# cserteGT3/RANSAC.jl

Measured on AMD Instinct MI355X. Metric: candidates_scored_per_sec, higher is better.
Workload: dtype f64; 1 GPU; cfg3: 10M-point 40-primitive cloud, 30% outliers, r=32 subsets, B=4096 candidates/GPU/step; points=10000000, subset_points=312500, score_mode=f64, parallelism=candidate-sharded x1, int32 sum all-reduce

## Files before the change

### include/ransac_hip.h

```cpp
#ifndef RANSAC_HIP_H
#define RANSAC_HIP_H

#include <stdint.h>

#ifdef __cplusplus
extern "C" {
#endif

#define RH_VERSION 121

enum {
    RH_OK = 0,
    RH_E_INVALID = -1,
    RH_E_NODEVICE = -2,
    RH_E_NOMEM = -3,
    RH_E_CAPACITY = -4,
    RH_E_INTERNAL = -5,
};

enum { RH_PLANE = 0, RH_SPHERE = 1, RH_CYLINDER = 2, RH_CONE = 3 };

typedef struct {
    int32_t kind;
    int32_t outwards;
    double v[10];
} rh_shape;

enum { RH_SCORE_INT64_WRAP = 0, RH_SCORE_F64 = 1 };
enum { RH_S_LENGTHC = 1, RH_S_ALLCAND = 2, RH_S_NOFMINSET = 3 };

typedef struct {
    double eps[4];
    double alpha[4];
    double cos_alpha[4];
    double collin_threshold;
    double parallelthrdeg;
    double cos_parallelthr;
    double sphere_par;
    double minconeopang;
    double prob_det;
    int64_t tau;
    int64_t itermax;
    int32_t drawN;
    int32_t minsubsetN;
    int32_t extract_s;
    int32_t terminate_s;
    int32_t n_shape_types;
    int32_t shape_types[8];
    int32_t score_mode;
    int32_t sphere_uses_enabled;
    int32_t sampling_streams;
    int32_t octree_sampling;
    int32_t octree_max_depth;
} rh_params;

typedef struct rh_cloud rh_cloud;

int rh_version(void);
const char *rh_last_error(void);
int rh_device_count(int *n_out);

void rh_default_params(rh_params *p);
void rh_params_finalize(rh_params *p);
void rh_shape_finalize(rh_shape *s);

int rh_cloud_create(const double *xyz_aos, const double *nrm_aos, int64_t n,
                    const int64_t *subset1_idx_1based, int64_t s, int device, rh_cloud **out);
int rh_cloud_create_f32(const float *xyz_aos, const float *nrm_aos, int64_t n,
                        const int64_t *subset1_idx_1based, int64_t s, int device, rh_cloud **out);
void rh_shape_finalize_f32(rh_shape *s);
int rh_cloud_destroy(rh_cloud *c);
int rh_cloud_info(const rh_cloud *c, int64_t *n, int64_t *s, int *device);
int rh_cloud_set_enabled(rh_cloud *c, const uint64_t *chunks, int64_t nchunks);
int rh_cloud_get_enabled(rh_cloud *c, uint64_t *chunks, int64_t nchunks);
int rh_cloud_enable_all(rh_cloud *c);
int rh_cloud_count_enabled(rh_cloud *c, int64_t *out);


int rh_score_batch(rh_cloud *c, const rh_shape *shapes, int32_t b, const rh_params *p,
                   int32_t *counts_out, uint64_t *masks_out_or_null);

int rh_score_batch_dev(rh_cloud *c, const rh_shape *d_shapes, int32_t b, const rh_params *p,
                       int32_t *d_counts, uint64_t *d_masks_or_null);

int rh_refit(rh_cloud *c, const rh_shape *shape, const rh_params *p,
             int64_t *idx_out_1based, int64_t cap, int64_t *n_out);

int rh_refit_component(rh_cloud *c, const rh_shape *shape, const rh_params *p, double beta, int32_t conn26,
                       int64_t *idx_out_1based, int64_t cap, int64_t *n_out,
                       int64_t *n_refit_out_or_null, int32_t *n_components_out_or_null);
int rh_cloud_set_component_filter(rh_cloud *c, double beta, int32_t conn26);
int rh_cloud_get_component_filter(const rh_cloud *c, double *beta_out, int32_t *conn26_out);
// ... 294 lines not shown
```

### include/ransac_hip_diag.h

```cpp
#ifndef RANSAC_HIP_DIAG_H
#define RANSAC_HIP_DIAG_H

#include "ransac_hip.h"

#ifdef __cplusplus
extern "C" {
#endif

int rh_dbg_cls_audit(rh_cloud *c, const rh_shape *shapes, int32_t b, const rh_params *p, double *out );
int rh_dbg_cls_soundness(rh_cloud *c, const rh_shape *shapes, int32_t b, const rh_params *p, uint64_t *out );
int rh_dbg_cls_soundness_tiles(rh_cloud *c, const rh_shape *shapes, int32_t b, const rh_params *p, uint64_t *out );
int rh_dbg_cls_soundness_nsig(rh_cloud *c, const rh_shape *shapes, int32_t b, const rh_params *p, uint64_t *out );
int rh_dbg_nsig(const rh_shape *shape, const rh_params *p, double M, double Nm, double Ln, int f32, uint32_t *mask_out ,
                const double *dirs, int64_t ndirs, int32_t *cells_out);
int rh_dbg_group_boxes(rh_cloud *c, double *out, int64_t cap, int64_t *ngroups_out);
int rh_dbg_cylbox(const rh_shape *shape, const rh_params *p, double M, double Nm, int f32, const double *boxes, int64_t n,
                  uint8_t *skip_out, uint8_t *ball_out, float *fields_out );
int rh_dbg_cls_round(const rh_shape *shape, const rh_params *p, double M, double Nm, int f32, int64_t n, const double *xyz,
                     const double *nrm, float *ua_out, float *ub_out, float *rec_out , double *dbg4_out );
int rh_dbg_books2(const float *u2, int64_t nseq, int32_t *sure_count_out, uint64_t *sure_word_out, uint64_t *und_word_out,
                  uint8_t *any_und_out);
int rh_dbg_cls_u2(const rh_shape *shape, const rh_params *p, double M, double Nm, int f32, int64_t n, const double *xyz,
                  const double *nrm, float *u_out, float *u2_out, float *rec_out );
int rh_dbg_conebox(const rh_shape *shape, const rh_params *p, double M, double Nm, int f32, const double *boxes, int64_t n,
                   uint8_t *skip_out, float *fields_out );
int rh_dbg_cls_cone(const rh_shape *shape, const rh_params *p, double M, double Nm, int f32, int64_t n, const double *xyz,
                    const double *nrm, int device, float *ua_out, float *ub_out, uint8_t *near_out, float *rec_out ,
                    double *dbg4_out );
int rh_dbg_oct_search_selftest(int64_t n, uint64_t seed, int64_t queries, int64_t *mismatches);

int rh_dbg_enabled_events(const uint8_t *events, int64_t nseq, int32_t len, uint16_t *answers);

int rh_dbg_s4_stats(rh_cloud *c, int mode, uint64_t *out );

typedef struct { int64_t slot; int32_t level; int32_t pad; rh_shape shape; } rh_dbg_cand;
int rh_dbg_sample_fit(rh_cloud *c, const rh_params *p, uint64_t seed, int64_t k0, int32_t n_iters, const double *P_or_null,
                      int32_t rank, int32_t world, rh_dbg_cand *out, int32_t cap, int32_t *n_out, uint64_t *draws_out,
                      int32_t *gave_up_out, int32_t *info_out );

int rh_dbg_wave_keys(const uint32_t *keys, const uint8_t *act, const int32_t *slot, int32_t n, int32_t nslots, int u32, int device,
                     int32_t *sum_out , int32_t *minlead_out , int32_t *scal_out );

#ifdef __cplusplus
}
#endif
#endif
```

### ransac.jl_amd/_lib.py

```python
import ctypes as C
import os

_HERE = os.path.dirname(os.path.abspath(__file__))
SO_PATH = os.path.join(_HERE, "libransac_hip.so")
SO_PATH_DIAG = os.path.join(_HERE, "libransac_hip_diag.so")
OPTION_UNSET = -(1 << 63)
SCORE_PATH = {"auto": 0, "brute": 1, "groups": 2}
REFIT_PATH = {"auto": 0, "scan": 1, "culled": 2}

PLANE, SPHERE, CYLINDER, CONE = 0, 1, 2, 3
KIND_NAMES = {PLANE: "plane", SPHERE: "sphere", CYLINDER: "cylinder", CONE: "cone"}
SCORE_INT64_WRAP, SCORE_F64 = 0, 1
S_LENGTHC, S_ALLCAND, S_NOFMINSET = 1, 2, 3
RH_OK, RH_E_INVALID, RH_E_NODEVICE, RH_E_NOMEM, RH_E_CAPACITY, RH_E_INTERNAL = 0, -1, -2, -3, -4, -5


class Shape(C.Structure):
    _fields_ = [("kind", C.c_int32), ("outwards", C.c_int32), ("v", C.c_double * 10)]


class Params(C.Structure):
    _fields_ = [
        ("eps", C.c_double * 4), ("alpha", C.c_double * 4), ("cos_alpha", C.c_double * 4),
        ("collin_threshold", C.c_double), ("parallelthrdeg", C.c_double), ("cos_parallelthr", C.c_double),
# ... 162 lines not shown
    "rh_shape_finalize_f32": (None, [C.POINTER(Shape)]),
    "rh_mp_open": (C.c_int, [C.c_char_p, C.c_int32, C.c_int32, C.c_int64, C.POINTER(_vp)]),
    "rh_mp_close": (C.c_int, [_vp]),
    "rh_mp_allgather": (C.c_int, [_vp, _vp, C.c_int64, _vp]),
    "rh_ransac_mp": (C.c_int, [_vp, C.POINTER(C.c_double), C.POINTER(C.c_double), C.POINTER(Params), C.POINTER(Rng), _vp, C.POINTER(Result)]),
    "rh_dev_free": (C.c_int, [_vp, _vp]),
    "rh_dev_upload": (C.c_int, [_vp, _vp, _vp, C.c_int64]),
    "rh_dev_download": (C.c_int, [_vp, _vp, _vp, C.c_int64]),
    "rh_octree_build": (C.c_int, [_dp, C.c_int64, C.POINTER(C.c_void_p)]),
    "rh_octree_build_f32": (C.c_int, [C.POINTER(C.c_float), C.c_int64, C.POINTER(C.c_void_p)]),
    "rh_octree_destroy": (C.c_int, [_vp]),
    "rh_octree_info": (C.c_int, [_vp, _i32p, _i32p, _i32p]),
    "rh_octree_findleaf": (C.c_int, [_vp, _dp, _i32p]),
    "rh_octree_getnthcell": (C.c_int, [_vp, C.c_int32, C.c_int32, _i32p]),
    "rh_octree_node_info": (C.c_int, [_vp, C.c_int32, _dp, _dp, _i32p, _i32p, _i32p, C.POINTER(C.c_int64)]),
    "rh_octree_node_points": (C.c_int, [_vp, C.c_int32, C.POINTER(C.c_int64), C.c_int64]),
    "rh_octree_cell_enabled": (C.c_int, [_vp, _vp, C.c_int32, C.POINTER(C.c_int64), C.c_int64, C.POINTER(C.c_int64)]),
    "rh_set_option": (C.c_int, [_vp, C.c_char_p, C.c_int64]),
    "rh_get_option": (C.c_int, [_vp, C.c_char_p, _i64p, _i32p]),
    "rh_score_launch_info": (C.c_int, [_vp, C.POINTER(C.c_int32)]),
    "rh_last_list_launch_ms": (C.c_int, [_vp, C.POINTER(C.c_float)]),
    "rh_build_variant": (C.c_int, []),
    "rh_cloud_create_ms": (C.c_int, [_vp, _dp]),
    "rh_comm_unique_id": (C.c_int, [_vp]),
    "rh_comm_create": (C.c_int, [_vp, C.c_int32, C.c_int32, _vp, C.POINTER(_vp)]),
    "rh_comm_destroy": (C.c_int, [_vp]),
    "rh_score_batch_allreduce_dev": (C.c_int, [_vp, _vp, _vp, C.c_int32, C.c_int32, C.c_int32, _pp, _vp]),
    "rh_comm_fence": (C.c_int, [_vp, _vp]),
    "rh_comm_sync": (C.c_int, [_vp]),
    "rh_shape_extents": (C.c_int, [_vp, _sp, C.c_int32, _i64p, _i64p, C.POINTER(Extent)]),
    "rh_shape_extents_dev": (C.c_int, [_vp, _vp, C.c_int32, _vp, _vp, C.c_int64, _vp]),
    "rh_result_extents": (C.c_int, [_vp, C.POINTER(Result), C.POINTER(Extent)]),
    "rh_assign_points": (C.c_int, [_dp, _dp, C.c_int64, _sp, C.c_int32, _pp, C.c_int32, C.c_int, _i32p, _dp, _i64p, _i64p, _i64p]),
    "rh_assign_points_f32": (C.c_int, [C.POINTER(C.c_float), C.POINTER(C.c_float), C.c_int64, _sp, C.c_int32, _pp, C.c_int32, C.c_int,
                                       _i32p, _dp, _i64p, _i64p, _i64p]),
    "rh_cloud_assign": (C.c_int, [_vp, _sp, C.c_int32, _pp, C.c_int32, _i32p, _dp, _i64p, _i64p, _i64p]),
    "rh_cloud_assign_dev": (C.c_int, [_vp, _vp, C.c_int32, _pp, C.c_int32, _vp, _vp, _vp, _vp, _vp]),
    "rh_estimate_normals": (C.c_int, [_dp, C.c_int64, C.POINTER(NormalsParams), _dp, C.c_int, _dp, _dp, _i32p]),
    "rh_estimate_normals_f32": (C.c_int, [C.POINTER(C.c_float), C.c_int64, C.POINTER(NormalsParams), C.POINTER(C.c_float),
                                          C.c_int, C.POINTER(C.c_float), C.POINTER(C.c_float), _i32p]),
    "rh_cluster": (C.c_int, [_dp, C.c_int64, C.POINTER(ClusterParams), C.c_int, _i32p, _u8p, C.c_int64, _i64p, _i64p, _i64p, _i64p,
                             C.POINTER(ClusterStats)]),
    "rh_cluster_f32": (C.c_int, [C.POINTER(C.c_float), C.c_int64, C.POINTER(ClusterParams), C.c_int, _i32p, _u8p, C.c_int64, _i64p,
                                 _i64p, _i64p, _i64p, C.POINTER(ClusterStats)]),
    "rh_orient_normals": (C.c_int, [_dp, _dp, C.c_int64, C.POINTER(OrientParams), C.c_int, _dp, _i32p, _i32p, C.POINTER(OrientStats)]),
    "rh_orient_normals_f32": (C.c_int, [C.POINTER(C.c_float), C.POINTER(C.c_float), C.c_int64, C.POINTER(OrientParams), C.c_int,
                                        C.POINTER(C.c_float), _i32p, _i32p, C.POINTER(OrientStats)]),
    "rh_voxel_downsample": (C.c_int, [_dp, _dp, C.c_int64, C.POINTER(VoxelParams), C.c_int, _dp, _dp, _i64p, _i32p, C.c_int64,
                                      _i32p, _i64p, _i64p]),
    "rh_voxel_downsample_f32": (C.c_int, [C.POINTER(C.c_float), C.POINTER(C.c_float), C.c_int64, C.POINTER(VoxelParams), C.c_int,
                                          C.POINTER(C.c_float), C.POINTER(C.c_float), _i64p, _i32p, C.c_int64, _i32p, _i64p, _i64p]),
    "rh_knn": (C.c_int, [_dp, C.c_int64, C.c_int32, C.c_double, C.c_int, _i32p, _dp, _i32p]),
    "rh_knn_f32": (C.c_int, [C.POINTER(C.c_float), C.c_int64, C.c_int32, C.c_double, C.c_int, _i32p, _dp, _i32p]),
    "rh_knn_query": (C.c_int, [_dp, C.c_int64, _dp, C.c_int64, C.c_int32, C.c_double, C.c_int, _i32p, _dp, _i32p]),
    "rh_knn_query_f32": (C.c_int, [C.POINTER(C.c_float), C.c_int64, C.POINTER(C.c_float), C.c_int64, C.c_int32, C.c_double, C.c_int,
                                   _i32p, _dp, _i32p]),
    "rh_cloud_distance": (C.c_int, [_dp, _dp, C.c_int64, _dp, C.c_int64, C.POINTER(DistanceParams), C.c_int, _dp, _i32p,
                                    C.POINTER(DistanceStats)]),
    "rh_cloud_distance_f32": (C.c_int, [C.POINTER(C.c_float), C.POINTER(C.c_float), C.c_int64, C.POINTER(C.c_float), C.c_int64,
                                        C.POINTER(DistanceParams), C.c_int, _dp, _i32p, C.POINTER(DistanceStats)]),
    "rh_register": (C.c_int, [_dp, _dp, C.c_int64, _dp, C.c_int64, C.POINTER(RegisterParams), _dp, C.c_int, _dp,
                              C.POINTER(RegisterResult), _i32p, _dp]),
    "rh_register_f32": (C.c_int, [C.POINTER(C.c_float), C.POINTER(C.c_float), C.c_int64, C.POINTER(C.c_float), C.c_int64,
                                  C.POINTER(RegisterParams), _dp, C.c_int, _dp, C.POINTER(RegisterResult), _i32p, _dp]),
    "rh_remove_outliers": (C.c_int, [_dp, C.c_int64, C.POINTER(OutlierParams), C.c_int, _u8p, _i32p, C.c_int64, _i64p, _dp,
                                     C.POINTER(OutlierStats)]),
    "rh_remove_outliers_f32": (C.c_int, [C.POINTER(C.c_float), C.c_int64, C.POINTER(OutlierParams), C.c_int, _u8p, _i32p,
                                         C.c_int64, _i64p, _dp, C.POINTER(OutlierStats)]),
}

class DbgCand(C.Structure):
    _fields_ = [("slot", C.c_int64), ("level", C.c_int32), ("pad", C.c_int32), ("shape", Shape)]


DIAG_SIGNATURES = {
    "rh_dbg_sample_fit": (C.c_int, [_vp, _pp, C.c_uint64, C.c_int64, C.c_int32, _dp, C.c_int32, C.c_int32, C.POINTER(DbgCand),
                                    C.c_int32, _i32p, _u64p, _i32p, _i32p]),
    "rh_dbg_cls_audit": (C.c_int, [_vp, _sp, C.c_int32, _pp, _dp]),
    "rh_dbg_cls_soundness": (C.c_int, [_vp, _sp, C.c_int32, _pp, C.POINTER(C.c_uint64)]),
    "rh_dbg_cls_soundness_tiles": (C.c_int, [_vp, _sp, C.c_int32, _pp, C.POINTER(C.c_uint64)]),
    "rh_dbg_cls_soundness_nsig": (C.c_int, [_vp, _sp, C.c_int32, _pp, C.POINTER(C.c_uint64)]),
    "rh_dbg_nsig": (C.c_int, [_sp, _pp, C.c_double, C.c_double, C.c_double, C.c_int, C.POINTER(C.c_uint32), _dp, C.c_int64, _i32p]),
    "rh_dbg_group_boxes": (C.c_int, [_vp, _dp, C.c_int64, C.POINTER(C.c_int64)]),
    "rh_dbg_cylbox": (C.c_int, [_sp, _pp, C.c_double, C.c_double, C.c_int, _dp, C.c_int64, C.POINTER(C.c_uint8), C.POINTER(C.c_uint8), C.POINTER(C.c_float)]),
    "rh_dbg_cls_round": (C.c_int, [_sp, _pp, C.c_double, C.c_double, C.c_int, C.c_int64, _dp, _dp, C.POINTER(C.c_float), C.POINTER(C.c_float),
                                   C.POINTER(C.c_float), _dp]),
    "rh_dbg_books2": (C.c_int, [C.POINTER(C.c_float), C.c_int64, _i32p, _u64p, _u64p, _u8p]),
    "rh_dbg_cls_u2": (C.c_int, [_sp, _pp, C.c_double, C.c_double, C.c_int, C.c_int64, _dp, _dp, C.POINTER(C.c_float), C.POINTER(C.c_float),
                                C.POINTER(C.c_float)]),
    "rh_dbg_conebox": (C.c_int, [_sp, _pp, C.c_double, C.c_double, C.c_int, _dp, C.c_int64, C.POINTER(C.c_uint8), C.POINTER(C.c_float)]),
    "rh_dbg_cls_cone": (C.c_int, [_sp, _pp, C.c_double, C.c_double, C.c_int, C.c_int64, _dp, _dp, C.c_int, C.POINTER(C.c_float),
                                  C.POINTER(C.c_float), C.POINTER(C.c_uint8), C.POINTER(C.c_float), _dp]),
    "rh_dbg_oct_search_selftest": (C.c_int, [C.c_int64, C.c_uint64, C.c_int64, C.POINTER(C.c_int64)]),
    "rh_dbg_enabled_events": (C.c_int, [_u8p, C.c_int64, C.c_int32, C.POINTER(C.c_uint16)]),
    "rh_dbg_s4_stats": (C.c_int, [_vp, C.c_int, C.POINTER(C.c_uint64)]),
    "rh_dbg_wave_keys": (C.c_int, [C.POINTER(C.c_uint32), _u8p, _i32p, C.c_int32, C.c_int32, C.c_int, C.c_int, _i32p, _i32p, _i32p]),
}

_libs = {}


def variant():
    v = os.environ.get("RH_LIB_VARIANT", "product")
    if v not in ("product", "diag"):
        raise RuntimeError("RH_LIB_VARIANT=%r: expected 'product' or 'diag'" % v)
    return v


def _share_torch_hip_runtime():
    import sys
    if "torch" in sys.modules or os.environ.get("RH_SYSTEM_HIP"):
        return
    try:
        import importlib.util
        spec = importlib.util.find_spec("torch")
        if spec is None or not spec.submodule_search_locations:
            return
        path = os.path.join(list(spec.submodule_search_locations)[0], "lib", "libamdhip64.so")
        if os.path.exists(path):
            C.CDLL(path, mode=C.RTLD_GLOBAL)
    except (ImportError, OSError, ValueError):
        pass


def lib(which=None):
    which = which or variant()
    L = _libs.get(which)
    if L is None:
        path = SO_PATH if which == "product" else SO_PATH_DIAG
        if os.environ.get("RH_LIB_PATH"):
            path = os.environ["RH_LIB_PATH"]
        if not os.path.exists(path):
            raise RuntimeError(
                "%s is missing: the HIP extension has not been built and this package has no CPU "
                "fallback (build it with ransac.jl_amd/build.py)" % path)
        _share_torch_hip_runtime()
        L = C.CDLL(path)
        sigs = dict(SIGNATURES)
        if which == "diag":
            sigs.update(DIAG_SIGNATURES)
        for name, (res, args) in sigs.items():
            f = getattr(L, name)
            f.restype = res
            f.argtypes = args
        if L.rh_build_variant() != (1 if which == "diag" else 0):
            raise RuntimeError("%s is not the %s build" % (path, which))
        _libs[which] = L
    return L


def check(rc):
    if rc != RH_OK:
        raise RansacHipError(rc, lib().rh_last_error().decode("utf-8", "replace"))
    return rc
```

### ransac.jl_amd/csrc/cloud.hip

```cpp
#include <functional>
#include <system_error>
#include <thread>
#include <stdarg.h>
#include <stdio.h>
#include <string.h>

#include <stdlib.h>

#include <algorithm>
#include <chrono>
#include <memory>
#include <new>
#include <utility>
#include <vector>

#include "rh_internal.h"
#include "score4_device.h"

static thread_local char g_err[512] = "";

void rh_set_error(const char *fmt, ...)
{
    va_list ap;
    va_start(ap, fmt);
// ... 376 lines not shown
                        code |= spread21((uint64_t)(t * 2097151.0)) << k;
                    }
                    keys[(size_t)j] = std::make_pair(code, (int32_t)j);
                }
                std::sort(keys.begin(), keys.end());
                for (int64_t i = 0; i < s; i++) order[(size_t)i] = keys[(size_t)i].second;
            } else {
                auto key = [&](int32_t j, int ax) {
                    const double v = xyz[3 * (subset1[j] - 1) + ax];
                    return v == v ? v : HUGE_VAL;
                };
                auto split = [&](int64_t lo_i, int64_t hi_i) -> int64_t {
                    const int64_t cnt = hi_i - lo_i;
                    if (cnt <= 64) return 0;
                    double blo[3] = { HUGE_VAL, HUGE_VAL, HUGE_VAL }, bhi[3] = { -HUGE_VAL, -HUGE_VAL, -HUGE_VAL };
                    for (int64_t i = lo_i; i < hi_i; i++) {
                        const double *pp = xyz + 3 * (subset1[order[(size_t)i]] - 1);
                        for (int k = 0; k < 3; k++) {
                            const double v = pp[k];
                            if (!(v == v) || v - v != 0) continue;
                            if (v < blo[k]) blo[k] = v;
                            if (v > bhi[k]) bhi[k] = v;
                        }
                    }
                    int ax = 0;
                    double best = -1;
                    for (int k = 0; k < 3; k++) {
                        const double e = bhi[k] - blo[k];
                        if (e > best) { best = e; ax = k; }
                    }
                    const int64_t nl = ((cnt / 64 + 1) / 2) * 64;
                    std::nth_element(order.begin() + lo_i, order.begin() + lo_i + nl, order.begin() + hi_i,
                                     [&](int32_t a, int32_t b) {
                                         const double ka = key(a, ax), kb = key(b, ax);
                                         return ka < kb || (ka == kb && a < b);
                                     });
                    return lo_i + nl;
                };
                struct Node { int64_t lo, hi; };
                auto subtree = [&](int64_t lo_i, int64_t hi_i) {
                    std::vector<Node> stack;
                    stack.push_back({ lo_i, hi_i });
                    while (!stack.empty()) {
                        const Node nd = stack.back();
                        stack.pop_back();
                        const int64_t mid = split(nd.lo, nd.hi);
                        if (mid == 0) continue;
                        stack.push_back({ mid, nd.hi });
                        stack.push_back({ nd.lo, mid });
                    }
                };
                constexpr int KD_PAR_LEVELS = 4;
                const unsigned hw = std::thread::hardware_concurrency();
                const int par_levels = (hw >= 16 ? KD_PAR_LEVELS : (hw >= 8 ? 3 : (hw >= 4 ? 2 : (hw >= 2 ? 1 : 0))));
                std::function<void(int64_t, int64_t, int)> build = [&](int64_t lo_i, int64_t hi_i, int depth) {
                    if (depth >= par_levels || hi_i - lo_i < 4096) { subtree(lo_i, hi_i); return; }
                    const int64_t mid = split(lo_i, hi_i);
                    if (mid == 0) return;
                    std::thread right;
                    try {
                        right = std::thread([&, mid, hi_i, depth]() { build(mid, hi_i, depth + 1); });
                    } catch (const std::system_error &) {
                        subtree(mid, hi_i);
                    }
                    build(lo_i, mid, depth + 1);
                    if (right.joinable()) right.join();
                };
                build(0, s, 0);
            }
            int32_t *h_perm = h_idx + s;
            for (int64_t i = 0; i < s; i++) {
                h_perm[i] = order[(size_t)i];
                h_idx[i] = (int32_t)(subset1[h_perm[i]] - 1);
            }
            ms_kd = ms_since(tkd0);
            CKH(hipMemcpyAsync(c->sub_idx0, h_idx, sizeof(int32_t) * (size_t)s, hipMemcpyHostToDevice, c->stream));
            CKH(hipMemcpyAsync(c->sub_perm, h_perm, sizeof(int32_t) * (size_t)s, hipMemcpyHostToDevice, c->stream));
            CK(rhk_transpose_aos(c, t_xyz, t_nrm, n, c->sub_idx0, s, c->sub, c->s_pad));
            CK(rhk_group_bounds(c));
            }
        }
    }
    stamp("subset order, gather, boxes");
    CK(rhk_enabled_replace(c, nullptr));
    CKH(hipStreamSynchronize(c->stream));
    stamp("enabled bits");
#undef CK
#undef CKH
    t_xyz.reset();
    t_nrm.reset();
    h_idx_own.reset();
    c->create_ms[0] = ms_since(tc0);
    c->create_ms[1] = ms_kd;
    c->create_ms[2] = ms_before_kd;
    c->create_ms[3] = c->create_ms[0] - ms_kd - ms_before_kd;
    *out = c;
    return RH_OK;
}

extern "C" int rh_cloud_create_ms(const rh_cloud *c, double *out4)
{
    if (!c || !out4) { rh_set_error("rh_cloud_create_ms: NULL argument"); return RH_E_INVALID; }
    for (int i = 0; i < 4; i++) out4[i] = c->create_ms[i];
    return RH_OK;
}

extern "C" int rh_cloud_destroy(rh_cloud *c)
{
    cloud_free(c);
    return RH_OK;
}

extern "C" int rh_cloud_create_f32(const float *xyz, const float *nrm, int64_t n, const int64_t *subset1, int64_t s, int device,
                                   rh_cloud **out)
{
    if (!out) { rh_set_error("out is NULL"); return RH_E_INVALID; }
    *out = nullptr;
    if (n < 0 || (n > 0 && (!xyz || !nrm))) { rh_set_error("rh_cloud_create_f32: bad arguments"); return RH_E_INVALID; }
    std::vector<double> x64((size_t)(3 * n)), n64((size_t)(3 * n));
    for (int64_t i = 0; i < 3 * n; i++) { x64[(size_t)i] = (double)xyz[i]; n64[(size_t)i] = (double)nrm[i]; }
    rh_cloud *c = nullptr;
    RH_TRY(rh_cloud_create(x64.data(), n64.data(), n, subset1, s, device, &c));
    c->f32 = true;
    c->f32_groups = c->use_groups;
    c->use_groups = false;
    int rc = c->full32.alloc(6 * std::max<int64_t>(c->n_pad, 1));
    if (rc == RH_OK) rc = c->sub32.alloc(6 * std::max<int64_t>(c->s_pad, 1));
    if (rc == RH_OK) rc = rhk_f32_build(c);
    if (rc == RH_OK && hipStreamSynchronize(c->stream) != hipSuccess) { rh_set_error("rh_cloud_create_f32: device error"); rc = RH_E_NODEVICE; }
    if (rc != RH_OK) { cloud_free(c); return rc; }
    *out = c;
    return RH_OK;
}

extern "C" int rh_cloud_info(const rh_cloud *c, int64_t *n, int64_t *s, int *device)
{
    if (!c) { rh_set_error("cloud is NULL"); return RH_E_INVALID; }
    if (n) *n = c->n;
    if (s) *s = c->s;
    if (device) *device = c->device;
    return RH_OK;
}

static int enter_nojoin(rh_cloud *c)
{
    if (!c) { rh_set_error("cloud is NULL"); return RH_E_INVALID; }
    RH_HIP(hipSetDevice(c->device));
    return RH_OK;
}

int rh_join_batches(rh_cloud *c)
{
    for (rh_batch_ws &w : c->ws) {
        if (w.dirty) RH_HIP(hipStreamWaitEvent(c->stream, w.done, 0));
        w.dirty = false;
        w.started = false;
        w.out_counts = nullptr;
        w.out_masks = nullptr;
    }
    c->pipe_k = 0;
    return RH_OK;
}

static int enter(rh_cloud *c)
{
    RH_TRY(enter_nojoin(c));
// ... 543 lines not shown
```

### ransac.jl_amd/csrc/enabled.hip

```cpp
#include "rh_internal.h"
#include "score_device.h"

namespace {

using namespace rhdev;

__global__ void __launch_bounds__(256)
block_popc_kernel(const uint64_t *__restrict__ words, int64_t nwords, int32_t *__restrict__ block_sums)
{
    __shared__ int32_t red[4];
    const int64_t base = (int64_t)blockIdx.x * RH_WORDS_PER_BLOCK;
    int acc = 0;
    for (int k = threadIdx.x; k < RH_WORDS_PER_BLOCK; k += 256) {
        const int64_t w = base + k;
        if (w < nwords) acc += __popcll(words[w]);
    }
    for (int off = 32; off > 0; off >>= 1) acc += __shfl_down(acc, off);
    if ((threadIdx.x & 63) == 0) red[threadIdx.x >> 6] = acc;
    __syncthreads();
    if (threadIdx.x == 0) block_sums[blockIdx.x] = red[0] + red[1] + red[2] + red[3];
}

__global__ void __launch_bounds__(1024)
scan_block_sums_kernel(int32_t *__restrict__ block_sums, int64_t nb, int32_t *__restrict__ total)
// ... 224 lines not shown
    sd[0] = r1;
    for (int i = 1; i < drawN; i++) {
        if (q >= L) return;
        int64_t pick = select(range(raw[q++], count));
        if (pick == sd[0]) {
            if (q >= L) return;
            pick = select(range(raw[q++], count));
        }
        sd[i] = pick;
    }
    bool distinct = true;
    for (int a = 1; a < drawN; a++)
        for (int b = 0; b < a; b++) distinct = distinct && sd[a] != sd[b];
    for (int i = 0; i < drawN; i++) o[i] = sd[i];
    o[drawN] = q - p;
    o[drawN + 1] = distinct ? 1 : 0;
}

__global__ void oct_gather_enabled_kernel(const uint64_t *__restrict__ enabled, const int32_t *__restrict__ perm,
                                          int64_t n, uint64_t *__restrict__ men)
{
    const int64_t j = (int64_t)blockIdx.x * blockDim.x + threadIdx.x;
    bool bit = false;
    if (j < n) {
        const int32_t i0 = perm[j];
        bit = (enabled[i0 >> 6] >> (i0 & 63)) & 1ULL;
    }
    const uint64_t w = __builtin_amdgcn_ballot_w64(bit);
    if ((threadIdx.x & 63) == 0 && (j >> 6) < (n + 63) / 64) men[j >> 6] = w;
}

}

static __global__ void __launch_bounds__(256)
expand_dense_kernel(const uint64_t *__restrict__ mask, int64_t nwords, const int32_t *__restrict__ word_prefix,
                    int32_t *__restrict__ out)
{
    const int64_t g = (int64_t)blockIdx.x * blockDim.x + threadIdx.x;
    const int64_t w = g >> 6;
    if (w >= nwords) return;
    const int lane = threadIdx.x & 63;
    const uint64_t m = mask[w];
    if ((m >> lane) & 1ULL) out[word_prefix[w] + __popcll(m & ((1ULL << lane) - 1ULL))] = (int32_t)g;
}

int rhk_enabled_alloc(rh_cloud *c)
{
    RH_TRY(c->enabled.alloc(c->nwords));
    RH_TRY(c->sub_enabled.alloc(c->swords));
    RH_TRY(c->d_ndis.alloc(1));
    RH_TRY(c->block_sums.alloc(std::max<int64_t>(c->nblocks, (c->swords + RH_WORDS_PER_BLOCK - 1) / RH_WORDS_PER_BLOCK) + 2));
    RH_TRY(c->en_block_sums.alloc(c->nblocks + 2));
    RH_TRY(c->word_prefix.alloc(c->nwords + 1));
    RH_TRY(c->d_total.alloc(1));
    RH_HIP(hipMemsetAsync(c->d_total, 0, sizeof(int32_t), c->stream));
    return RH_OK;
}

rh_scan_scratch rhk_take_scan_scratch(rh_cloud *c) { c->en.scratch_taken(); return { c->block_sums.get(), c->d_total.get() }; }
const int32_t *rhk_fold_total(const rh_cloud *c) { return c->d_total; }
void rhk_enabled_run_ended(rh_cloud *c) { c->en.scratch_taken(); }

int rhk_compact_generic(hipStream_t stream, const uint64_t *mask, int64_t nwords, int32_t *ws_block_sums,
                        int64_t *idx_out, int64_t cap, int32_t *d_total, int32_t *word_prefix_out)
{
    const int64_t nb = (nwords + RH_WORDS_PER_BLOCK - 1) / RH_WORDS_PER_BLOCK;
    if (nb > 0) hipLaunchKernelGGL(block_popc_kernel, dim3((unsigned)nb), dim3(256), 0, stream, mask, nwords, ws_block_sums);
    hipLaunchKernelGGL(scan_block_sums_kernel, dim3(1), dim3(1024), 0, stream, ws_block_sums, nb, d_total);
    if (nb > 0)
        hipLaunchKernelGGL(expand_mask_kernel, dim3((unsigned)nb), dim3(256), 0, stream, mask, nwords, ws_block_sums,
                           idx_out, cap, word_prefix_out, (uint64_t *)nullptr, (int32_t *)nullptr);
    RH_HIP(hipGetLastError());
    return RH_OK;
}

static int rebuild_sub_enabled(rh_cloud *c, bool reset_list)
{
    if (reset_list) RH_HIP(hipMemsetAsync(c->d_ndis, 0, sizeof(int32_t), c->stream));
    if (c->s == 0) return RH_OK;
    hipLaunchKernelGGL(update_sub_enabled_kernel, dim3(cdiv(c->swords, 4 * RH_SUBUPD_WPW)), dim3(256), 0, c->stream,
                       c->enabled, c->sub_idx0, c->s, c->swords, c->sub_enabled, reset_list ? 1 : 0, c->sub, c->s_pad,
                       c->dis, c->dis_stride, c->d_ndis);
    RH_HIP(hipGetLastError());
    return RH_OK;
}

static int read_ndis(rh_cloud *c)
{
    int32_t ndis = 0;
    RH_HIP(hipMemcpyAsync(&ndis, c->d_ndis, sizeof ndis, hipMemcpyDeviceToHost, c->stream));
    RH_HIP(hipStreamSynchronize(c->stream));
    c->n_dis = ndis;
    return RH_OK;
}

int rhk_enabled_replace(rh_cloud *c, const uint64_t *chunks)
{
    const bool all = chunks == nullptr;
    const bool mirror = all && c->k_built && c->nwords > 0;
    if (c->nwords > 0) {
        if (all) RH_HIP(hipMemsetAsync(c->enabled, 0xFF, sizeof(uint64_t) * (size_t)c->nwords, c->stream));
        else RH_HIP(hipMemcpyAsync(c->enabled, chunks, sizeof(uint64_t) * (size_t)c->nwords, hipMemcpyHostToDevice, c->stream));
        if (c->n % 64) {
            const uint64_t last = (all ? ~0ULL : chunks[c->nwords - 1]) & ((~0ULL) >> (64 - c->n % 64));
            RH_HIP(hipMemcpyAsync(c->enabled + (c->nwords - 1), &last, sizeof last, hipMemcpyHostToDevice, c->stream));
        }
        if (!all || c->n % 64) RH_HIP(hipStreamSynchronize(c->stream));
        if (mirror) RH_HIP(hipMemcpyAsync(c->oct_men, c->enabled, sizeof(uint64_t) * (size_t)c->nwords, hipMemcpyDeviceToDevice, c->stream));
    }
    c->en.bits_replaced(mirror);
    RH_TRY(rebuild_sub_enabled(c, true));
    c->n_dis = 0;
    return all ? RH_OK : read_ndis(c);
}

int rhk_enabled_clear_list(rh_cloud *c, const int64_t *d_idx, int64_t n)
{
    if (n == 0) return RH_OK;
    const bool both = c->k_built && c->en.has_mirror();
    hipLaunchKernelGGL(invalidate_idx_kernel, dim3(cdiv(n, 256)), dim3(256), 0, c->stream, d_idx, n, c->n, c->enabled,
                       both ? c->oct_pos : (const int32_t *)nullptr, both ? c->oct_men : (uint64_t *)nullptr);
    RH_HIP(hipGetLastError());
    c->en.bits_cleared_by_list(both);
    RH_TRY(rebuild_sub_enabled(c, false));
    return read_ndis(c);
}

int rhk_enabled_apply_refit(rh_cloud *c)
{
    if (c->nblocks > 0 && !c->en.scan_left_sums())
        hipLaunchKernelGGL(block_popc_kernel, dim3((unsigned)c->nblocks), dim3(256), 0, c->stream, c->refit_mask, c->nwords,
                           c->block_sums);
    const bool raw = c->nblocks > 0 && c->nblocks <= 2048;
    if (!raw) hipLaunchKernelGGL(scan_block_sums_kernel, dim3(1), dim3(1024), 0, c->stream, c->block_sums, c->nblocks, c->d_total);
    if (c->nblocks > 0)
        hipLaunchKernelGGL(expand_mask_kernel, dim3((unsigned)c->nblocks), dim3(256), 0, c->stream, c->refit_mask, c->nwords,
                           c->block_sums, c->idx_out, c->n, (int32_t *)nullptr, c->enabled, c->en_block_sums,
                           raw ? c->d_total : (int32_t *)nullptr);
    RH_HIP(hipGetLastError());
    c->en.scan_folded(c->nblocks > 0);
    return rebuild_sub_enabled(c, false);
}

int rhk_enabled_resync(rh_cloud *c)
{
    c->en.scratch_taken();
    RH_TRY(rebuild_sub_enabled(c, true));
    return read_ndis(c);
}

int rhk_ensure_select(rh_cloud *c)
{
    if (c->en.has_directory()) return RH_OK;
    if (c->nwords > 0) {
        if (!c->en.has_block_sums())
            hipLaunchKernelGGL(block_popc_kernel, dim3((unsigned)c->nblocks), dim3(256), 0, c->stream, c->enabled, c->nwords,
                               c->en_block_sums);
        hipLaunchKernelGGL(scan_block_sums_kernel, dim3(1), dim3(1024), 0, c->stream, c->en_block_sums, c->nblocks, c->d_total);
        hipLaunchKernelGGL(expand_mask_kernel, dim3((unsigned)c->nblocks), dim3(256), 0, c->stream, c->enabled, c->nwords,
                           c->en_block_sums, (int64_t *)nullptr, (int64_t)0, c->word_prefix, (uint64_t *)nullptr,
                           (int32_t *)nullptr);
        RH_HIP(hipGetLastError());
    }
    c->en.directory_built();
    return RH_OK;
}

// ... 95 lines not shown
```

### ransac.jl_amd/csrc/kdorder.hip

```cpp
#include <stdlib.h>

#include <algorithm>
#include <vector>

#include <hipcub/hipcub.hpp>

#include "rh_internal.h"

namespace {

inline unsigned cdivq(int64_t a, int64_t b) { return (unsigned)((a + b - 1) / b); }

__device__ __forceinline__ uint32_t ord32(float v)
{
    const uint32_t b = __builtin_bit_cast(uint32_t, v);
    if ((b & 0x7fffffffu) > 0x7f800000u) return 0xffffffffu;
    return (b & 0x80000000u) ? ~b : (b | 0x80000000u);
}
__device__ __forceinline__ float unord32(uint32_t u)
{
    const uint32_t b = (u & 0x80000000u) ? (u & 0x7fffffffu) : ~u;
    return __builtin_bit_cast(float, b);
}

__global__ void __launch_bounds__(256)
kd_gather_kernel(const double *__restrict__ xyz, const double *__restrict__ nrm, const int32_t *__restrict__ idx0, int64_t s,
                 float *__restrict__ px, float *__restrict__ py, float *__restrict__ pz, int32_t *__restrict__ ord,
                 unsigned long long *__restrict__ mags)
{
    const int64_t j = (int64_t)blockIdx.x * blockDim.x + threadIdx.x;
    double cm = 0.0, nm = 0.0;
    if (j < s) {
        const int64_t i = idx0[j];
        const double x = xyz[3 * i], y = xyz[3 * i + 1], z = xyz[3 * i + 2];
        px[j] = (float)x; py[j] = (float)y; pz[j] = (float)z;
        ord[j] = (int32_t)j;
        const double v[6] = { x, y, z, nrm[3 * i], nrm[3 * i + 1], nrm[3 * i + 2] };
#pragma unroll
        for (int k = 0; k < 6; k++) {
            const double a = fabs(v[k]);
            if (a - a == 0) { if (k < 3) cm = a > cm ? a : cm; else nm = a > nm ? a : nm; }
        }
    }
    for (int off = 32; off > 0; off >>= 1) {
        const double oc = __shfl_xor(cm, off), on = __shfl_xor(nm, off);
        cm = oc > cm ? oc : cm;
        nm = on > nm ? on : nm;
    }
    if ((threadIdx.x & 63) == 0) {
        if (cm > 0) atomicMax(&mags[0], __builtin_bit_cast(unsigned long long, cm));
        if (nm > 0) atomicMax(&mags[1], __builtin_bit_cast(unsigned long long, nm));
    }
}

__device__ __forceinline__ int seg_of(const int32_t *__restrict__ seg_lo, int nseg, int32_t i)
{
    int lo = 0, hi = nseg;
    while (hi - lo > 1) {
        const int mid = (lo + hi) >> 1;
        if (seg_lo[mid] <= i) lo = mid; else hi = mid;
    }
    return lo;
}

__global__ void __launch_bounds__(256)
kd_box_kernel(const float *__restrict__ px, const float *__restrict__ py, const float *__restrict__ pz, const int32_t *__restrict__ ord,
              int64_t s, const int32_t *__restrict__ seg_lo, const uint8_t *__restrict__ seg_active, int nseg, uint32_t *__restrict__ box)
{
    const int64_t i = (int64_t)blockIdx.x * blockDim.x + threadIdx.x;
    const bool in = i < s;
    const int seg = in ? seg_of(seg_lo, nseg, (int32_t)i) : -1;
    const bool act = in && seg_active[seg] != 0;
    uint32_t mn[3] = { 0xffffffffu, 0xffffffffu, 0xffffffffu }, mx[3] = { 0u, 0u, 0u };
    if (act) {
        const int32_t j = ord[i];
        const float v[3] = { px[j], py[j], pz[j] };
#pragma unroll
        for (int k = 0; k < 3; k++)
            if (v[k] - v[k] == 0.0f) { mn[k] = mx[k] = ord32(v[k]); }
    }
    const int seg0 = __shfl(seg, 0);
    const bool uniform = __builtin_amdgcn_ballot_w64(seg != seg0) == 0;
    if (uniform) {
        if (seg0 < 0 || !__shfl((int)act, 0)) return;
#pragma unroll
        for (int k = 0; k < 3; k++)
            for (int off = 32; off > 0; off >>= 1) {
                const uint32_t a = __shfl_xor(mn[k], off), b = __shfl_xor(mx[k], off);
                mn[k] = a < mn[k] ? a : mn[k];
                mx[k] = b > mx[k] ? b : mx[k];
            }
        if ((threadIdx.x & 63) == 0) {
#pragma unroll
            for (int k = 0; k < 3; k++) { atomicMin(&box[seg0 * 6 + k], mn[k]); atomicMax(&box[seg0 * 6 + 3 + k], mx[k]); }
        }
    } else if (act) {
#pragma unroll
        for (int k = 0; k < 3; k++) { atomicMin(&box[seg * 6 + k], mn[k]); atomicMax(&box[seg * 6 + 3 + k], mx[k]); }
    }
}

__global__ void __launch_bounds__(256)
kd_key_kernel(const float *__restrict__ px, const float *__restrict__ py, const float *__restrict__ pz, const int32_t *__restrict__ ord,
              int64_t s, const int32_t *__restrict__ seg_lo, const uint8_t *__restrict__ seg_active, int nseg,
              const uint32_t *__restrict__ box, uint64_t *__restrict__ keys)
{
    const int64_t i = (int64_t)blockIdx.x * blockDim.x + threadIdx.x;
    if (i >= s) return;
    const int seg = seg_of(seg_lo, nseg, (int32_t)i);
    uint32_t sub = (uint32_t)i;
    if (seg_active[seg] != 0) {
        int ax = 0;
        float best = -2.0f;
#pragma unroll
        for (int k = 0; k < 3; k++) {
            const uint32_t lo = box[seg * 6 + k], hi = box[seg * 6 + 3 + k];
            const float e = lo <= hi ? unord32(hi) - unord32(lo) : -1.0f;
            if (e > best) { best = e; ax = k; }
        }
        const int32_t j = ord[i];
        sub = ord32(ax == 0 ? px[j] : (ax == 1 ? py[j] : pz[j]));
    }
    keys[i] = ((uint64_t)(uint32_t)seg << 32) | sub;
}

__global__ void kd_fill_box_kernel(uint32_t *__restrict__ box, int nseg)
{
    const int t = blockIdx.x * blockDim.x + threadIdx.x;
    if (t < nseg * 6) box[t] = (t % 6) < 3 ? 0xffffffffu : 0u;
}

__global__ void kd_finish_kernel(const int32_t *__restrict__ ord, const int32_t *__restrict__ idx0, int64_t s,
                                 int32_t *__restrict__ sub_perm, int32_t *__restrict__ sub_idx0)
{
    const int64_t i = (int64_t)blockIdx.x * blockDim.x + threadIdx.x;
    if (i >= s) return;
    const int32_t j = ord[i];
    sub_perm[i] = j;
    sub_idx0[i] = idx0[j];
}

struct KdNode { int32_t lo, hi; };

__device__ __forceinline__ unsigned long long ord64(double v)
{
    const unsigned long long b = __builtin_bit_cast(unsigned long long, v);
    return (b >> 63) ? ~b : (b | 0x8000000000000000ULL);
}
__global__ void __launch_bounds__(256)
aabb_kernel(const double *__restrict__ xyz, int64_t n, unsigned long long *__restrict__ out)
{
    unsigned long long mn[3] = { ~0ULL, ~0ULL, ~0ULL }, mx[3] = { 0ULL, 0ULL, 0ULL };
    double mag = 0.0;
    for (int64_t i = (int64_t)blockIdx.x * blockDim.x + threadIdx.x; i < n; i += (int64_t)gridDim.x * blockDim.x) {
#pragma unroll
        for (int k = 0; k < 3; k++) {
            const double a = xyz[3 * i + k];
            if (a == a) {
                const unsigned long long o = ord64(a);
                mn[k] = o < mn[k] ? o : mn[k];
                mx[k] = o > mx[k] ? o : mx[k];
                const double m = fabs(a);
                if (m - m == 0 && m > mag) mag = m;
            }
        }
    }
    unsigned long long mb = __builtin_bit_cast(unsigned long long, mag);
    for (int off = 32; off > 0; off >>= 1) {
#pragma unroll
        for (int k = 0; k < 3; k++) {
            const unsigned long long a = __shfl_xor(mn[k], off), b = __shfl_xor(mx[k], off);
            mn[k] = a < mn[k] ? a : mn[k];
            mx[k] = b > mx[k] ? b : mx[k];
        }
        const unsigned long long c = __shfl_xor(mb, off);
        mb = c > mb ? c : mb;
    }
    if ((threadIdx.x & 63) == 0) {
#pragma unroll
        for (int k = 0; k < 3; k++) { atomicMin(&out[k], mn[k]); atomicMax(&out[3 + k], mx[k]); }
        atomicMax(&out[6], mb);
    }
}

}

int rhk_cloud_aabb(rh_cloud *c, const double *d_xyz, int64_t n, double lo[3], double hi[3], bool has[3], double *mag)
{
    for (int k = 0; k < 3; k++) { lo[k] = hi[k] = 0; has[k] = false; }
    *mag = 0;
    if (n <= 0) return RH_OK;
    unsigned long long h[7];
    rh_dev<unsigned long long> d;
    RH_TRY(d.alloc(7));
    for (int k = 0; k < 7; k++) h[k] = k < 3 ? ~0ULL : 0ULL;
    RH_HIP(hipMemcpyAsync(d, h, sizeof h, hipMemcpyHostToDevice, c->stream));
    hipLaunchKernelGGL(aabb_kernel, dim3((unsigned)std::min<int64_t>(4096, (n + 255) / 256)), dim3(256), 0, c->stream, d_xyz, n, d.get());
    RH_HIP(hipGetLastError());
    RH_HIP(hipMemcpyAsync(h, d, sizeof h, hipMemcpyDeviceToHost, c->stream));
    RH_HIP(hipStreamSynchronize(c->stream));
    auto un = [](unsigned long long u) { const unsigned long long b = (u >> 63) ? (u & 0x7fffffffffffffffULL) : ~u; return __builtin_bit_cast(double, b); };
    for (int k = 0; k < 3; k++) {
        has[k] = h[k] <= h[3 + k];
        if (has[k]) { lo[k] = un(h[k]); hi[k] = un(h[3 + k]); }
    }
    *mag = __builtin_bit_cast(double, h[6]);
    return RH_OK;
}

int rhk_kd_order(rh_cloud *c, const double *d_xyz, const double *d_nrm, const int32_t *d_idx0)
{
    const int64_t s = c->s;
    if (s <= 0) return RH_OK;
    if (s > (int64_t)0x7fffffff) { rh_set_error("rhk_kd_order: subset of %lld points", (long long)s); return RH_E_INVALID; }
    rh_dev<float> pf;
    rh_dev<int32_t> ord[2], seg_lo;
    rh_dev<uint64_t> keys[2];
    rh_dev<uint32_t> box;
    rh_dev<uint8_t> seg_act;
    rh_dev<unsigned long long> mags;
    rh_dev<char> tmp;
    size_t tmp_bytes = 0;
    std::vector<std::vector<KdNode>> levels;
    {
        std::vector<KdNode> cur(1, KdNode{ 0, (int32_t)s });
        for (;;) {
            bool any = false;
            for (const KdNode &nd : cur) any = any || nd.hi - nd.lo > 64;
            if (!any) break;
            levels.push_back(cur);
            std::vector<KdNode> nxt;
            nxt.reserve(cur.size() * 2);
            for (const KdNode &nd : cur) {
                const int32_t cnt = nd.hi - nd.lo;
                if (cnt <= 64) { nxt.push_back(nd); continue; }
                const int32_t nl = ((cnt / 64 + 1) / 2) * 64;
                nxt.push_back(KdNode{ nd.lo, nd.lo + nl });
                nxt.push_back(KdNode{ nd.lo + nl, nd.hi });
            }
            cur.swap(nxt);
        }
    }
    size_t max_seg = 1;
    for (const auto &lv : levels) max_seg = std::max(max_seg, lv.size());
    RH_TRY(pf.alloc(3 * s));
    RH_TRY(ord[0].alloc(s));
    RH_TRY(ord[1].alloc(s));
    RH_TRY(keys[0].alloc(s));
    RH_TRY(keys[1].alloc(s));
    RH_TRY(box.alloc(6 * (int64_t)max_seg));
    RH_TRY(mags.alloc(2));
    RH_HIP(hipMemsetAsync(mags, 0, sizeof(unsigned long long) * 2, c->stream));
    float *px = pf, *py = pf + s, *pz = pf + 2 * s;
    const dim3 gs(cdivq(s, 256)), blk(256);
    hipLaunchKernelGGL(kd_gather_kernel, gs, blk, 0, c->stream, d_xyz, d_nrm, d_idx0, s, px, py, pz, ord[0], mags);
    RH_HIP(hipGetLastError());
    RH_HIP(hipcub::DeviceRadixSort::SortPairs(nullptr, tmp_bytes, keys[0].get(), keys[1].get(), ord[0].get(), ord[1].get(), (int)s, 0, 64, c->stream));
    RH_TRY(tmp.alloc((int64_t)tmp_bytes));
    std::vector<int32_t> h_lo;
    std::vector<uint8_t> h_act;
    std::vector<size_t> off_lo, off_act;
    for (const auto &lv : levels) {
        off_lo.push_back(h_lo.size());
        off_act.push_back(h_act.size());
        for (const KdNode &nd : lv) { h_lo.push_back(nd.lo); h_act.push_back(nd.hi - nd.lo > 64 ? 1 : 0); }
        h_lo.push_back((int32_t)s);
    }
    RH_TRY(seg_lo.alloc((int64_t)h_lo.size()));
    RH_TRY(seg_act.alloc((int64_t)h_act.size()));
    if (!h_lo.empty()) RH_HIP(hipMemcpyAsync(seg_lo, h_lo.data(), sizeof(int32_t) * h_lo.size(), hipMemcpyHostToDevice, c->stream));
    if (!h_act.empty()) RH_HIP(hipMemcpyAsync(seg_act, h_act.data(), h_act.size(), hipMemcpyHostToDevice, c->stream));
    int cur = 0;
    for (size_t L = 0; L < levels.size(); L++) {
        const int nseg = (int)levels[L].size();
        const int32_t *lo_l = seg_lo + off_lo[L];
        const uint8_t *act_l = seg_act + off_act[L];
        hipLaunchKernelGGL(kd_fill_box_kernel, dim3(cdivq((int64_t)nseg * 6, 256)), blk, 0, c->stream, box, nseg);
        hipLaunchKernelGGL(kd_box_kernel, gs, blk, 0, c->stream, px, py, pz, ord[cur], s, lo_l, act_l, nseg, box);
        hipLaunchKernelGGL(kd_key_kernel, gs, blk, 0, c->stream, px, py, pz, ord[cur], s, lo_l, act_l, nseg, box, keys[0]);
        RH_HIP(hipGetLastError());
        int seg_bits = 1;
        while ((1 << seg_bits) < nseg) seg_bits++;
        RH_HIP(hipcub::DeviceRadixSort::SortPairs(tmp.get(), tmp_bytes, keys[0].get(), keys[1].get(), ord[cur].get(), ord[cur ^ 1].get(), (int)s, 0, 32 + seg_bits, c->stream));
        cur ^= 1;
    }
    hipLaunchKernelGGL(kd_finish_kernel, gs, blk, 0, c->stream, ord[cur], d_idx0, s, c->sub_perm, c->sub_idx0);
    RH_HIP(hipGetLastError());
    unsigned long long h_mags[2] = { 0, 0 };
    RH_HIP(hipMemcpyAsync(h_mags, mags, sizeof h_mags, hipMemcpyDeviceToHost, c->stream));
    RH_HIP(hipStreamSynchronize(c->stream));
    c->coord_mag = __builtin_bit_cast(double, h_mags[0]);
    c->nrm_mag = __builtin_bit_cast(double, h_mags[1]);
    return RH_OK;
}
```

### ransac.jl_amd/csrc/options.cpp

```cpp
#include <stdlib.h>
#include <string.h>

#include "rh_internal.h"

namespace {

enum { T_INT = 0, T_FLAG = 1, T_ENUM_SCORE = 2, T_ENUM_REFIT = 3, T_ENUM_ORDER = 4 };

struct OptDef {
    int id;
    const char *key;
#ifdef RH_DIAG
    const char *env;
#endif
    int type;
};

#ifdef RH_DIAG
#define RH_O(id, key, env, type) { id, key, env, type }
#else
#define RH_O(id, key, env, type) { id, key, type }
#endif

const OptDef kDefs[] = {
    RH_O(RH_OPT_SCORE_PATH, "score_path", "RH_SCORE_PATH", T_ENUM_SCORE),
    RH_O(RH_OPT_S4_ROWS, "s4_rows", "RH_S4_R", T_INT),
    RH_O(RH_OPT_UNP_WORDS, "unp_words", "RH_UNP_WORDS", T_INT),
    RH_O(RH_OPT_ST_CULL, "st_cull", "RH_ST_CULL", T_INT),
    RH_O(RH_OPT_REFIT_PATH, "refit_path", "RH_REFIT_PATH", T_ENUM_REFIT),
    RH_O(RH_OPT_BATCHES_IN_FLIGHT, "batches_in_flight", "RH_BATCHES_IN_FLIGHT", T_INT),
    RH_O(RH_OPT_ST_LIST_MB, "st_list_mb", "RH_ST_LIST_MB", T_INT),
    RH_O(RH_OPT_NSIG, "nsig", "RH_NSIG", T_INT),
#ifdef RH_DIAG
    RH_O(RH_OPT_CREATE_PROF, "create_prof", "RH_CREATE_PROF", T_FLAG),
    RH_O(RH_OPT_AABB_HOST, "aabb_host", "RH_AABB_HOST", T_FLAG),
    RH_O(RH_OPT_SUB_ORDER, "sub_order", "RH_SUB_ORDER", T_ENUM_ORDER),
    RH_O(RH_OPT_KD_HOST, "kd_host", "RH_KD_HOST", T_FLAG),
    RH_O(RH_OPT_NO_SPREAD, "no_spread", "RH_NO_SPREAD", T_FLAG),
    RH_O(RH_OPT_OCT_CHAIN_W, "oct_chain_w", "RH_OCT_CHAIN_W", T_INT),
    RH_O(RH_OPT_NO_MANAGED_STORE, "no_managed_store", "RH_NO_MANAGED_STORE", T_FLAG),
    RH_O(RH_OPT_OCT_ONE_WINDOW, "oct_one_window", "RH_OCT_ONE_WINDOW", T_FLAG),
    RH_O(RH_OPT_OCT_WINDOW_ITERS, "oct_window_iters", "RH_OCT_WINDOW_ITERS", T_INT),
    RH_O(RH_OPT_NO_FUSED_SCORE, "no_fused_score", "RH_NO_FUSED_SCORE", T_FLAG),
    RH_O(RH_OPT_NO_PIPELINE, "no_pipeline", "RH_NO_PIPELINE", T_FLAG),
    RH_O(RH_OPT_NO_OCT_CHAIN, "no_oct_chain", "RH_NO_OCT_CHAIN", T_FLAG),
    RH_O(RH_OPT_REFIT_BLOCKS, "refit_blocks", "RH_REFIT_BLOCKS", T_INT),
    RH_O(RH_OPT_NO_FUSED_SAMPLER, "no_fused_sampler", "RH_NO_FUSED_SAMPLER", T_FLAG),
    RH_O(RH_OPT_NO_CREC, "no_crec", "RH_NO_CREC", T_FLAG),
    RH_O(RH_OPT_LONG_WINDOW_SETS, "long_window_sets", "RH_LONG_WINDOW_SETS", T_INT),
    RH_O(RH_OPT_NO_OCT_TAB, "no_oct_tab", "RH_NO_OCT_TAB", T_FLAG),
    RH_O(RH_OPT_NO_DRIVER_CACHE, "no_driver_cache", "RH_NO_DRIVER_CACHE", T_FLAG),
    RH_O(RH_OPT_HOST_SAMPLER, "host_sampler", "RH_HOST_SAMPLER", T_FLAG),
    RH_O(RH_OPT_DRIVER_PROF, "driver_prof", "RH_DRIVER_PROF", T_FLAG),
    RH_O(RH_OPT_G2_DBG, "g2_dbg", "RH_G2_DBG", T_INT),
    RH_O(RH_OPT_KREFIT_DBG, "krefit_dbg", "RH_KREFIT_DBG", T_FLAG),
    RH_O(RH_OPT_NO_FAST_EXTRACT, "no_fast_extract", "RH_NO_FAST_EXTRACT", T_FLAG),
#endif
};
constexpr int kNDefs = (int)(sizeof(kDefs) / sizeof(kDefs[0]));

int64_t g_opt[RH_OPT_COUNT];
bool g_init = false;

void init_once()
{
    if (g_init) return;
    for (int i = 0; i < RH_OPT_COUNT; i++) g_opt[i] = RH_OPTION_UNSET;
    g_init = true;
}

const OptDef *find_key(const char *key)
{
    if (key == nullptr) return nullptr;
    for (int i = 0; i < kNDefs; i++)
        if (strcmp(kDefs[i].key, key) == 0) return &kDefs[i];
    return nullptr;
}

#ifdef RH_DIAG
int64_t parse_env(const OptDef &d, const char *e)
{
    switch (d.type) {
    case T_FLAG: return 1;
    case T_ENUM_SCORE: return e[0] == 'b' ? RH_SCORE_PATH_BRUTE : (e[0] == 'g' ? RH_SCORE_PATH_GROUPS : RH_OPTION_UNSET);
    case T_ENUM_REFIT: return e[0] == 's' ? RH_REFIT_PATH_SCAN : (e[0] == 'c' ? RH_REFIT_PATH_CULLED : RH_OPTION_UNSET);
    case T_ENUM_ORDER: return e[0] == 'm' ? 1 : 0;
    default: return (int64_t)atoll(e);
    }
}
#endif

}

int64_t rh_opt(const rh_cloud *c, int id)
{
    if (id < 0 || id >= RH_OPT_COUNT) return RH_OPTION_UNSET;
    init_once();
    if (c != nullptr && c->opt[id] != RH_OPTION_UNSET) return c->opt[id];
    if (g_opt[id] != RH_OPTION_UNSET) return g_opt[id];
#ifdef RH_DIAG
    for (int i = 0; i < kNDefs; i++)
        if (kDefs[i].id == id) {
            const char *e = getenv(kDefs[i].env);
            return e != nullptr ? parse_env(kDefs[i], e) : RH_OPTION_UNSET;
        }
#endif
    return RH_OPTION_UNSET;
}

#ifdef RH_DIAG
const char *rh_opt_env_string(const char *name) { return getenv(name); }
#endif

void rh_opt_init_cloud(rh_cloud *c)
{
    for (int i = 0; i < RH_OPT_COUNT; i++) c->opt[i] = RH_OPTION_UNSET;
}

extern "C" int rh_build_variant(void)
{
#ifdef RH_DIAG
    return 1;
#else
    return 0;
#endif
}

extern "C" int rh_set_option(rh_cloud *c, const char *key, int64_t value)
{
    init_once();
    const OptDef *d = find_key(key);
    if (d == nullptr) { rh_set_error("rh_set_option: unknown option '%s'", key ? key : "(null)"); return RH_E_INVALID; }
    if (value != RH_OPTION_UNSET) {
        bool ok = true;
        switch (d->id) {
        case RH_OPT_SCORE_PATH: ok = value >= 0 && value <= RH_SCORE_PATH_GROUPS; break;
        case RH_OPT_REFIT_PATH: ok = value >= 0 && value <= RH_REFIT_PATH_CULLED; break;
        case RH_OPT_S4_ROWS: ok = value == 0 || value == 1 || value == 2 || value == 4 || value == 8 || value == 12 || value == 16; break;
        case RH_OPT_UNP_WORDS: ok = value >= 0 && value <= 16384; break;
        case RH_OPT_ST_CULL: ok = value >= 0 && value <= 2; break;
        case RH_OPT_BATCHES_IN_FLIGHT: ok = value >= 0 && value <= RH_MAX_IN_FLIGHT; break;
        case RH_OPT_ST_LIST_MB: ok = value >= 0 && value <= (1 << 20); break;
        case RH_OPT_NSIG: ok = value == 0 || value == 2; break;
        default: break;
        }
        if (!ok) { rh_set_error("rh_set_option: value %lld is not valid for '%s'", (long long)value, key); return RH_E_INVALID; }
    }
    if (d->id == RH_OPT_SCORE_PATH && c != nullptr) {
        rh_set_error("rh_set_option: 'score_path' is fixed when a cloud is created (its point order depends on it): set it process-wide (cloud = NULL) before rh_cloud_create");
        return RH_E_INVALID;
    }
    if (c != nullptr) {
        if (d->id == RH_OPT_BATCHES_IN_FLIGHT) { const int rc = rh_cloud_join(c); if (rc != RH_OK) return rc; }
        c->opt[d->id] = value;
    } else {
        g_opt[d->id] = value;
    }
    return RH_OK;
}

extern "C" int rh_get_option(const rh_cloud *c, const char *key, int64_t *value_out, int32_t *is_set)
{
    const OptDef *d = find_key(key);
    if (d == nullptr || value_out == nullptr) { rh_set_error("rh_get_option: unknown option '%s'", key ? key : "(null)"); return RH_E_INVALID; }
    const int64_t v = rh_opt(c, d->id);
    *value_out = v == RH_OPTION_UNSET ? 0 : v;
    if (is_set != nullptr) *is_set = v != RH_OPTION_UNSET;
    return RH_OK;
}
```

### ransac.jl_amd/csrc/rh_internal.h

```cpp
#pragma once

#include <hip/hip_runtime.h>
#include <stdint.h>

#include <vector>

#include "ransac_hip.h"
#include "dev_buf.h"
#include "enabled_state.h"

void rh_set_error(const char *fmt, ...);

#define RH_HIP(call)                                                                        \
    do {                                                                                    \
        hipError_t e_ = (call);                                                             \
        if (e_ != hipSuccess) {                                                             \
            rh_set_error("%s failed: %s (%s:%d)", #call, hipGetErrorString(e_), __FILE__,   \
                         __LINE__);                                                         \
            return RH_E_NODEVICE;                                                           \
        }                                                                                   \
    } while (0)

#define RH_TRY(call)                 \
    do {                             \
        int rc_ = (call);            \
        if (rc_ != RH_OK) return rc_; \
    } while (0)

static inline int cdiv(int64_t a, int64_t b) { return (int)((a + b - 1) / b); }

enum rh_opt_id {
    RH_OPT_SCORE_PATH = 0,
    RH_OPT_S4_ROWS,
    RH_OPT_UNP_WORDS,
    RH_OPT_ST_CULL,
    RH_OPT_REFIT_PATH,
    RH_OPT_BATCHES_IN_FLIGHT,
    RH_OPT_ST_LIST_MB,
    RH_OPT_NSIG,
    RH_OPT_N_PRODUCT,
    RH_OPT_CREATE_PROF = RH_OPT_N_PRODUCT, RH_OPT_AABB_HOST, RH_OPT_SUB_ORDER, RH_OPT_KD_HOST, RH_OPT_NO_SPREAD, RH_OPT_OCT_CHAIN_W,
    RH_OPT_NO_MANAGED_STORE, RH_OPT_OCT_ONE_WINDOW, RH_OPT_OCT_WINDOW_ITERS, RH_OPT_NO_FUSED_SCORE, RH_OPT_NO_PIPELINE,
    RH_OPT_NO_OCT_CHAIN, RH_OPT_REFIT_BLOCKS, RH_OPT_NO_FUSED_SAMPLER, RH_OPT_NO_CREC, RH_OPT_LONG_WINDOW_SETS, RH_OPT_NO_OCT_TAB,
    RH_OPT_NO_DRIVER_CACHE, RH_OPT_HOST_SAMPLER, RH_OPT_DRIVER_PROF, RH_OPT_G2_DBG, RH_OPT_KREFIT_DBG, RH_OPT_NO_FAST_EXTRACT,
    RH_OPT_COUNT
};
struct rh_cloud;
int64_t rh_opt(const rh_cloud *c, int id);
void rh_opt_init_cloud(rh_cloud *c);
#ifdef RH_DIAG
const char *rh_opt_env_string(const char *name);
static inline bool rh_opt_on(const rh_cloud *c, int id) { const int64_t v = rh_opt(c, id); return v != RH_OPTION_UNSET && v != 0; }
static inline int64_t rh_opt_int(const rh_cloud *c, int id, int64_t dflt) { const int64_t v = rh_opt(c, id); return v == RH_OPTION_UNSET ? dflt : v; }
#else
static inline bool rh_opt_on(const rh_cloud *c, int id) { if (id >= RH_OPT_N_PRODUCT) return false; const int64_t v = rh_opt(c, id); return v != RH_OPTION_UNSET && v != 0; }
static inline int64_t rh_opt_int(const rh_cloud *c, int id, int64_t dflt) { if (id >= RH_OPT_N_PRODUCT) return dflt; const int64_t v = rh_opt(c, id); return v == RH_OPTION_UNSET ? dflt : v; }
#endif

struct rh_prep {
    double f[12];
};

__host__ __device__ inline void prep_derived(rh_prep &o, int kind)
{
    o.f[11] = (((((fabs(o.f[0]) + fabs(o.f[1])) + fabs(o.f[2])) + fabs(o.f[3])) + fabs(o.f[4])) + fabs(o.f[5])) + fabs(o.f[6]);
    if (kind == RH_CYLINDER) {
        const double a2 = (o.f[0] * o.f[0] + o.f[1] * o.f[1]) + o.f[2] * o.f[2];
        const double k = 2.0 - a2;
        o.f[8] = (1.0 + fabs(o.f[3])) + (fabs(o.f[4]) + fabs(o.f[5]));
        o.f[9] = k;
        o.f[10] = 1.0 + fabs(k) * a2;
    }
}

__host__ __device__ __forceinline__ void prep_one(const rh_shape &s, rh_prep &o)
{
#pragma unroll
    for (int i = 0; i < 12; i++) o.f[i] = 0.0;
    const double sgn = s.outwards ? 1.0 : -1.0;
    switch (s.kind) {
    case RH_PLANE: {
        for (int i = 0; i < 6; i++) o.f[i] = s.v[i];
        const double a = s.v[3], b = s.v[4], c = s.v[5];
        const double inv = 1.0 / sqrt((a * a + b * b) + c * c);
        o.f[6] = inv * a; o.f[7] = inv * b; o.f[8] = inv * c;
        break;
    }
    case RH_SPHERE:
        for (int i = 0; i < 4; i++) o.f[i] = s.v[i];
        o.f[4] = sgn;
        break;
    case RH_CYLINDER:
        for (int i = 0; i < 7; i++) o.f[i] = s.v[i];
        o.f[7] = sgn;
        break;
    default:
        for (int i = 0; i < 6; i++) o.f[i] = s.v[i];
        o.f[6] = s.v[7];
        o.f[7] = s.v[8];
        o.f[8] = sgn;
        break;
    }
    prep_derived(o, s.kind);
}
inline void rh_prep_host(const rh_shape &s, rh_prep *out) { prep_one(s, *out); }

struct rh_prepf {
    float f[12];
};
template <int KIND>
__host__ __device__ inline rh_prepf prepf_of(const rh_prep &P)
{
    rh_prepf o;
    for (int i = 0; i < 9; i++) o.f[i] = (float)P.f[i];
    for (int i = 9; i < 12; i++) o.f[i] = 0.0f;
    if (KIND == RH_PLANE) {
        const float a = o.f[3], b = o.f[4], c = o.f[5];
        const float inv = 1.0f / sqrtf((a * a + b * b) + c * c);
        o.f[6] = inv * a; o.f[7] = inv * b; o.f[8] = inv * c;
    }
    if (KIND == RH_SPHERE) { o.f[5] = o.f[6] = o.f[7] = o.f[8] = 0.0f; }
    if (KIND == RH_CYLINDER) { o.f[8] = 0.0f; }
// ... 48 lines not shown
    int64_t mstride4 = 0;
    bool masks4 = false;
    rh_dev<uint16_t> d_stlist;
    rh_dev<int32_t> d_stcount;
    int64_t stlist_cap = 0, stlist_nst = 0;
    int64_t stlist_nomem = 0;
    rh_dev<uint64_t> d_segmask;
    int64_t segmask_words = 0;
};
struct rh_bins {
    const rh_prep *prep[4];
    const int32_t *orig[4];
    const void *cls[4];
    const float *box[4];
};
static inline rh_bins rh_bins_at(const rh_prep *prep, const int32_t *orig, const void *cls, const float *box, const int64_t off[4])
{
    rh_bins B;
    for (int k = 0; k < 4; k++) {
        B.prep[k] = prep + off[k];
        B.orig[k] = orig + off[k];
        B.cls[k] = cls ? (const char *)cls + (size_t)off[k] * 64 : nullptr;
        B.box[k] = box ? box + off[k] : nullptr;
    }
    return B;
}
static inline rh_bins rh_ws_bins(const rh_batch_ws &w)
{
    const int64_t off[4] = { 0, w.batch_cap, 2 * w.batch_cap, 3 * w.batch_cap };
    return rh_bins_at(w.d_prep, w.d_orig, w.d_qpre, w.d_box, off);
}
struct rh_score_job {
    rh_bins bins = {};
    int64_t bstride = 0;
    const uint64_t *en[4] = { nullptr, nullptr, nullptr, nullptr };
    const int32_t *nk[4] = { nullptr, nullptr, nullptr, nullptr };
    int32_t bound = 0;
    int32_t kind_bound[4] = { 0, 0, 0, 0 };
    const double *eps = nullptr, *cosa = nullptr;
    int32_t *d_counts = nullptr;
    uint64_t *d_masks_int = nullptr;
    rh_s4_points points = { nullptr, 0, 0, 0, nullptr };
    const int32_t *stop = nullptr;
    bool open_count = false;
    hipEvent_t ev_listed = nullptr;
};
struct rh_cloud {
    int64_t opt[RH_OPT_COUNT];
    int device = -1;
    hipStream_t stream = nullptr;
    hipStream_t own_stream = nullptr;
    hipEvent_t ev0 = nullptr, ev1 = nullptr;
    hipEvent_t evk[5] = { nullptr, nullptr, nullptr, nullptr, nullptr };
    hipStream_t copy_stream = nullptr;
    hipEvent_t ev_copied = nullptr;
    hipEvent_t ev_sync = nullptr;
    int64_t n = 0, s = 0;
    int64_t n_pad = 0, s_pad = 0;
    int64_t nwords = 0, swords = 0;
    int64_t nblocks = 0;

    rh_dev<double> full;
    rh_dev<double> set_ws;
    rh_dev<int32_t> set_level;
    int64_t set_ws_sets = 0;
    rh_dev<double> rec;
    rh_dev<double> sub;
    rh_dev<int32_t> sub_idx0;
    rh_dev<int32_t> sub_perm;
    rh_dev<double> gb;
    int64_t ngroups = 0, ng_pad = 0;
    double create_ms[4] = { 0, 0, 0, 0 };
    double coord_mag = 0;
    double nrm_mag = 0;
    bool use_groups = false;
    rh_dev<float> gb32;
    rh_dev<float> st32;
    int64_t nst = 0;
    rh_dev<float> tile32;
    int64_t ntile = 0;
    rh_dev<uint32_t> gm32;
    rh_dev<uint32_t> stm32;
    double nrm_len = 0;
    rh_dev<double> dis_gb;

    rh_enabled_state en;
    rh_dev<uint64_t> enabled;
    rh_dev<uint64_t> sub_enabled;
    rh_dev<double> dis;
    int64_t dis_stride = 0;
    rh_dev<int32_t> d_ndis;
    int64_t n_dis = 0;
    rh_dev<uint64_t> oct_men;
    rh_dev<int32_t> oct_prefix;
    rh_dev<int32_t> en_block_sums;
    rh_dev<int32_t> word_prefix;
    rh_dev<int32_t> sel_list;
    rh_dev<double> crec;
    rh_dev<int32_t> block_sums;
    rh_dev<int32_t> d_total;

    bool k_built = false;
    double k_lo[3] = { 0, 0, 0 }, k_size = 1;
    double k_mag = 0;
    rh_dev<double> fullk;
    rh_dev<float> fullk32;
    rh_dev<double> kgb;
    int64_t kg_pad = 0;
    rh_dev<int32_t> klist;
    rh_dev<int32_t> kctr;
    rh_dev<uint8_t> kflag;
    bool oct_built = false;
    int oct_depth = 0, oct_max_depth = 0;
    rh_dev<uint64_t> oct_code;
    rh_dev<int32_t> oct_perm;
    rh_dev<int32_t> oct_pos;
    rh_dev<rh_oct_state> oct_state;
    rh_dev<float> dis_gb32;
    rh_dev<unsigned long long> s4_stats;
    rh_dev<int32_t> oct_adv_tab;
    rh_dev<unsigned long long> oct_adv_bits;
    int64_t oct_adv_cells = 0;
    rh_dev<double> oct_adv_E;
    rh_dev<uint64_t> oct_code_o;
    rh_dev<int32_t> oct_tab;
    int oct_tab_level = 0;
    rh_dev<double> oct_P;
    std::vector<uint64_t> h_oct_code;
    std::vector<int32_t> h_oct_perm, h_oct_pos;

    rh_dev<uint64_t> refit_mask;
    rh_dev<int64_t> idx_out;

    double comp_beta = 0;
    int32_t comp_conn26 = 1;
    rh_dev<char> comp_tab;
    int64_t comp_cap = 0;
    rh_dev<uint64_t> comp_scal;
    rh_pinned<uint64_t> comp_h;

    rh_dev<double> ext_part;
    int64_t ext_part_rows = 0;
    rh_dev<int32_t> ext_flag;
    rh_dev<char> ext_in;

    rh_dev<char> asg_ws;
    rh_dev<char> asg_io;

    rh_batch_ws ws[RH_MAX_IN_FLIGHT];
    uint32_t pipe_k = 0;

    rh_dev<int32_t> d_nk;
    rh_dev<uint64_t> d_masks;
    rh_dev<int32_t> d_zero;
    hipEvent_t ev_cull = nullptr;
    float last_cull_ms = 0.f;
    int32_t last_s4[4] = { 0, 0, 0, 0 };

    rh_dev<int64_t> d_ranks;

    bool f32 = false;
    bool f32_groups = false;
    rh_dev<float> full32;
    rh_dev<float> sub32;

    int32_t mp_rank = 0, mp_world = 1;
#ifdef RH_DIAG
    int32_t dbg_sampler_path[6] = { 0, 0, 0, 0, 0, 0 };
#endif

    void *drv_cache = nullptr;
    void (*drv_cache_free)(rh_cloud *, void *) = nullptr;

    rh_dev<char> d_stage;

    rh_pinned<char> h_pin;
};

static inline rh_score_job rh_subset_job(const rh_cloud *c, const rh_params *p, const rh_bins &bins, int64_t bstride, const int32_t *d_nk)
{
    rh_score_job J;
    J.bins = bins;
    J.bstride = bstride;
    for (int k = 0; k < 4; k++) {
        J.en[k] = (k == RH_SPHERE && !p->sphere_uses_enabled) ? nullptr : c->sub_enabled.get();
        J.nk[k] = d_nk + k;
    }
    J.eps = p->eps;
    J.cosa = p->cos_alpha;
    return J;
}

struct rh_live_args {
    const rh_prep *prep[4];
    int32_t nk[4], base[4];
    int64_t first[4];
    double eps[4], cosa[4];
    int32_t f32 = 0;
};

int rhk_transpose_aos(rh_cloud *c, const double *d_aos_xyz, const double *d_aos_nrm, int64_t n,
                      const int32_t *d_gather_or_null, int64_t count, double *dst, int64_t dst_stride);
int rhk_fetch2_i32(rh_cloud *c, const int32_t *d_src0, const int32_t *d_src1, int32_t *h_pinned_dst);
int rhk_pack_records(rh_cloud *c, const double *d_xyz, const double *d_nrm, int64_t n, double *d_rec);
int rhk_prep_sorted(rh_cloud *c, rh_batch_ws &w, int32_t b, int32_t *d_counts_to_zero = nullptr, const double *eps = nullptr,
                    const double *cosa = nullptr);
int rhk_prep_records(rh_cloud *c, const rh_shape *d_shapes, int32_t b, rh_prep *d_prep);
struct rh_cand_entry;
struct rh_oct_state;
int rhk_prep_entries(rh_cloud *c, rh_batch_ws &w, const rh_cand_entry *d_entries, const int32_t *d_count, int32_t cap_entries,
                     int32_t launch_bound, int32_t *d_counts, int nk_is_zero, const double *eps = nullptr,
                     const double *cosa = nullptr, const rh_oct_state *ost = nullptr);
int rhk_prep_binned(rh_cloud *c, rh_batch_ws &w, const rh_shape *d_shapes, int32_t b, int32_t *d_nk, int32_t *d_counts_to_zero,
                    int32_t *d_nk_other, int nk_is_zero, const double *eps = nullptr, const double *cosa = nullptr,
                    int32_t *zero_extra = nullptr, int32_t zero_extra_n = 0);
bool rh_score_v4_enabled(const rh_cloud *c);
int rhk_score4_all(rh_cloud *c, rh_batch_ws &w, const rh_score_job &job, int32_t *launch_info = nullptr);
int rhk_unpermute_masks4(rh_cloud *c, rh_batch_ws &w, int32_t b, uint64_t *d_out);
int rhk_score_kind(rh_cloud *c, int kind, const double *pts, int64_t stride, int64_t s,
                   const uint64_t *enabled_words_or_null, const rh_prep *d_prep, const int32_t *d_orig,
                   const int32_t *d_nk, int32_t nk_bound, double eps, double cosa, int32_t *d_counts,
                   uint64_t *d_masks_or_null, int64_t mask_stride);
int rhk_score_kind(rh_cloud *c, int kind, const float *pts, int64_t stride, int64_t s,
                   const uint64_t *enabled_words_or_null, const rh_prep *d_prep, const int32_t *d_orig,
                   const int32_t *d_nk, int32_t nk_bound, double eps, double cosa, int32_t *d_counts,
                   uint64_t *d_masks_or_null, int64_t mask_stride);
int rhk_gb32_build(rh_cloud *c);
int rhk_store_cls(rh_cloud *c, const rh_prep *const prep[4], const int32_t n[4], const int32_t pbase[5], const double eps[4],
                  const double cosa[4], void *d_cls, float *d_box, int64_t bstride);
int rhk_score4_dis(rh_cloud *c, int64_t first, int64_t cnt, rh_score_job job);
int rhk_cloud_aabb(rh_cloud *c, const double *d_xyz, int64_t n, double lo[3], double hi[3], bool has[3], double *mag);
int rhk_kd_order(rh_cloud *c, const double *d_xyz, const double *d_nrm, const int32_t *d_idx0);
int rhk_score_kind_dis(rh_cloud *c, int kind, int64_t first, int64_t cnt, const rh_prep *d_prep, const int32_t *d_orig,
                       const int32_t *d_nk, int32_t nk_bound, double eps, double cosa, int32_t *d_counts);
int rhk_group_bounds(rh_cloud *c);
int rhk_unpermute_masks(rh_cloud *c, const uint64_t *d_in, int32_t b, uint64_t *d_out);
int rhk_refit_mask(rh_cloud *c, const rh_prep &P, int kind, double eps, double cosa, bool apply = false);
int rhk_korder_build(rh_cloud *c, const double *d_xyz, const double *d_nrm, const double lo[3], double size, double mag);
int rhk_f32_build(rh_cloud *c);
bool rhk_refit_is_culled(const rh_cloud *c);
int rhk_refitk_mask(rh_cloud *c, const rh_prep &P, int kind, double eps, double cosa, bool apply);
int rhk_group_bounds_of(rh_cloud *c, const double *pts, int64_t stride, int64_t count, int64_t ngroups, double *gb, int64_t gstride);
int rhk_oct_build_tab(rh_cloud *c);
int rhk_component_filter(rh_cloud *c, double beta, int conn26, int64_t *n_refit_out);
int rhk_component_stats(rh_cloud *c, int64_t *h_ncomp);
int rhk_liveness_small(rh_cloud *c, int64_t lo, int64_t span, const rh_live_args &A, int32_t *d_flags);
int rhk_pack_live(rh_cloud *c, int32_t *d_flags, int32_t n_flags, int32_t *h_flags, int32_t *h_scalars);
uint64_t rh_rng_next_raw(rh_rng *r);
int rhk_iota(rh_cloud *c, int32_t *d, int32_t n, int32_t base);
int rhk_gather_prep(rh_cloud *c, const rh_prep *src, const int32_t *d_idx, int32_t n, rh_prep *dst);
constexpr int RH_STORE_PAD = 256;
struct rh_store_plan {
    const rh_prep *prep[4];
    rh_prep *spare[4];
    const int32_t *id[4];
    int32_t *spare_id[4];
    const double *E[4];
    double *spare_E[4];
    int32_t n[4], pbase[5];
    const int32_t *counts;
    int32_t extracted_id;
};
struct rh_store_best { double E; long long id; };
int rhk_store_compact(rh_cloud *c, const rh_store_plan &P, int32_t *d_work, int32_t *h_out, int32_t *h_dead, rh_store_best *h_best,
                      int32_t *d_dead, rh_store_best *d_best);

int rhk_compact_generic(hipStream_t stream, const uint64_t *mask, int64_t nwords, int32_t *ws_block_sums,
                        int64_t *idx_out, int64_t cap, int32_t *d_total, int32_t *word_prefix_out = nullptr);

int rhk_enabled_alloc(rh_cloud *c);
int rhk_enabled_replace(rh_cloud *c, const uint64_t *chunks);
int rhk_enabled_clear_list(rh_cloud *c, const int64_t *d_idx, int64_t n);
int rhk_enabled_apply_refit(rh_cloud *c);
int rhk_enabled_resync(rh_cloud *c);
void rhk_enabled_run_ended(rh_cloud *c);
const int32_t *rhk_fold_total(const rh_cloud *c);
struct rh_scan_scratch { int32_t *sums, *total; };
rh_scan_scratch rhk_take_scan_scratch(rh_cloud *c);
int rhk_refit_total(rh_cloud *c, const char *who, int64_t *host_out, int64_t cap, int64_t *total_out, hipEvent_t ev = nullptr);
int rhk_ensure_select(rh_cloud *c);
int rhk_build_sel_list(rh_cloud *c);
int rhk_enabled_total(rh_cloud *c, int32_t *count);
int rhk_select(rh_cloud *c, const int64_t *d_ranks, int32_t k, int64_t *d_out);
int rhk_sample_sets_seq(rh_cloud *c, const uint64_t *d_raw, int32_t L, int32_t drawN, int64_t *d_rec);
int rhk_count_enabled(rh_cloud *c, int64_t *out);
int rhk_korder_sync_enabled(rh_cloud *c);
int rhk_oct_sync_enabled(rh_cloud *c);

struct rh_cand_entry {
    int64_t slot;
    int32_t level;
    int32_t pad;
    rh_shape shape;
};
struct rh_oct_state {
    double S[32], P[32];
    double best_E;
    long long store_count, cc2;
    rh_prep *store_prep[4];
    double *store_E[4];
    int32_t *store_id[4];
    long long store_cap[4];
    long long appended;
    int32_t store_n[4];
    int32_t has_best;
    int32_t stop;
    int32_t start;
    int32_t it_done;
};
int rhk_sample_fit(rh_cloud *c, const rh_params *prm, uint64_t seed, int64_t k0, int32_t n_iters, int32_t n_enabled,
                   const double *d_P, rh_cand_entry *d_out, int32_t cap, void *d_status, int status_is_zero,
                   int32_t *d_nk_zero, int32_t it0 = 0, const rh_oct_state *ost = nullptr);
struct rh_oct_iter_hdr {
    int32_t skipped;
    int32_t overflow;
// ... 29 lines not shown
```

### ransac.jl_amd/csrc/score4.hip

```cpp
#include <stdio.h>
#include <stdlib.h>

#include <vector>

#include "rh_internal.h"
#ifdef RH_DIAG
#include "ransac_hip_diag.h"
#endif
#include "score_device.h"
#include "score4_device.h"
#include "wave_keys.h"

namespace {

using namespace rhdev;
using namespace rh4;

typedef float rh_f32x4 __attribute__((ext_vector_type(4)));
typedef float rh_f32x2 __attribute__((ext_vector_type(2)));
typedef unsigned long long rh_u64x2 __attribute__((ext_vector_type(2)));
typedef uint32_t rh_u32x4 __attribute__((ext_vector_type(4)));

constexpr int S4_TG = 4;
constexpr int S4_GB = 2;
constexpr unsigned S4_GM = (1u << S4_GB) - 1u;
constexpr int S4_ROW = 65;
constexpr int S4_W = 4;
constexpr int S4_STG = 16;
template <int R, bool MASK = false, bool LIST = false>
struct S4Shared {
    static_assert(S4_TG == (1 << S4_GB) && R * 64 * S4_TG <= 65536 && (R % S4_W == 0 || R < S4_W), "entry encoding: S4_GB bits of group, the rest of 16 for the candidate");
    rh_f32x4 pa[S4_TG][S4_ROW];
    rh_f32x2 pb[S4_TG][S4_ROW];
    uint64_t len[S4_TG];
    rh_f32x4 gbox[S4_TG][2];
    rh_u32x4 gmask[S4_TG];
    uint16_t plist[R * 64 * S4_TG + 2];
    uint16_t ctab[LIST ? R * 64 : 2];
    int32_t cntb[S4_W][64];
    unsigned long long maskb[S4_W][64];
    uint16_t qb[S4_W][128];
    int weirdw[S4_TG];
    int npairs, next_batch;
};

static __device__ __forceinline__ bool is_nan_bits(float v)
{
    return (__builtin_bit_cast(uint32_t, v) & 0x7fffffffu) > 0x7f800000u;
}

struct S4KindArgs {
    const rh_cls *cls;
    const float *box;
    const rh_prep *prep;
    const int32_t *orig, *nk;
    const uint64_t *en;
    double eps, cosa;
};
struct S4AllArgs {
    const int32_t *stop;
    int row0;
    int rows;
    S4KindArgs k[4];
    int64_t ntiles, bstride, ngroups;
    const float *gb32;
    const uint32_t *gm32;
    uint64_t *masks;
    uint8_t *occ;
    int64_t mstride;
    unsigned long long *stats;
    const uint16_t *stlist;
    const int32_t *stcount;
    int64_t stcap;
};

#ifdef RH_DIAG
#define S4_STAT(stats, idx, val) do { const unsigned long long v_ = (unsigned long long)(val); if ((stats) != nullptr && (threadIdx.x & 63) == 0) atomicAdd((stats) + (idx), v_); } while (0)
#else
#define S4_STAT(stats, idx, val) do { } while (0)
#endif

template <int KIND> struct S4Fields { static constexpr int NBOX = KIND == RH_PLANE ? 8 : (KIND == RH_SPHERE ? 5 : (KIND == RH_CYLINDER ? 10 : 11)); };

static __device__ __forceinline__ bool nsig_meet(const float (&B)[RH_BOX_FIELDS], const rh_u32x4 gm)
{
    return (((__builtin_bit_cast(uint32_t, B[5]) & gm.x) | (__builtin_bit_cast(uint32_t, B[6]) & gm.y)) | (__builtin_bit_cast(uint32_t, B[7]) & gm.z)) != 0u;
}

#define RH4_CONST_AS __attribute__((address_space(4)))

static __device__ __forceinline__ int wave_shr1(int v) { return __builtin_amdgcn_update_dpp(0, v, 0x138, 0xf, 0xf, false); }
static __device__ __forceinline__ int wave_shl1(int v) { return __builtin_amdgcn_update_dpp(0, v, 0x130, 0xf, 0xf, false); }

static __device__ __forceinline__ int run_total(int v, int key, int lane)
{
    static_assert(S4_TG <= 4, "two steps cover runs of four");
    const int k1 = wave_shr1(key), u1 = wave_shr1(v);
    v += (lane >= 1 && k1 == key) ? u1 : 0;
    const int k2 = wave_shr1(k1), u2 = wave_shr1(wave_shr1(v));
    v += (lane >= 2 && k2 == key) ? u2 : 0;
    const int kn = wave_shl1(key);
    return (lane == 63 || kn != key) ? v : 0;
}

template <int KIND, int R, bool MASK, bool F32, bool LIST>
static __device__ __forceinline__ void
score4_batch(S4Shared<R, MASK, LIST> &sh, const int wv, const int lane, const int head, const int n, const int cbase, const double *__restrict__ pts,
             int64_t stride, const int64_t p0, const rh_prep *__restrict__ prep, const rh_cls *__restrict__ cls,
             const int32_t *__restrict__ orig, double eps, double cosa, int32_t *__restrict__ counts, const bool weird,
             uint64_t *__restrict__ masks, uint8_t *__restrict__ occ, const int64_t mstride, const int64_t g0, unsigned long long *__restrict__ stats)
{
    (void)stats;
    S4_STAT(stats, 24 * KIND + 8, 1);
    const bool act = lane < n;
    const uint32_t e = sh.plist[head + (act ? lane : 0)];
    const int g = (int)(e & S4_GM), ci = LIST ? (int)sh.ctab[e >> S4_GB] : cbase + (int)(e >> S4_GB);
    const rh_f32x4 *__restrict__ rowa = &sh.pa[g][0];
    const rh_f32x2 *__restrict__ rowb = &sh.pb[g][0];
    const rh_cls *__restrict__ rec = &cls[ci];
    int total = 0;
    uint64_t word = 0;
    int qbh = 0, qbn = 0;
    auto drain_b = [&](int k) {
        wave_lds_sync();
        const bool on = lane < k;
        const unsigned e2 = on ? sh.qb[wv][(qbh + lane) & 127] : 0u;
        const int slot = (int)(e2 >> 6);
        const uint32_t pe = sh.plist[head + slot];
        const int64_t gi = p0 + (int)(pe & S4_GM) * 64 + (int)(e2 & 63u);
        uint64_t r;
        if (F32) {
            const rh_prepf Pv = prepf_of<KIND>(prep[LIST ? (int)sh.ctab[pe >> S4_GB] : cbase + (int)(pe >> S4_GB)]);
            const rh_f32x4 a = sh.pa[pe & S4_GM][e2 & 63u];
            const rh_f32x2 b = sh.pb[pe & S4_GM][e2 & 63u];
            r = test_point<KIND>(Pv, a.x, a.y, a.z, a.w, b.x, b.y, eps, cosa);
        } else {
            const rh_prep Pv = prep[LIST ? (int)sh.ctab[pe >> S4_GB] : cbase + (int)(pe >> S4_GB)];
            r = test_point<KIND>(Pv, pts[gi], pts[stride + gi], pts[2 * stride + gi], pts[3 * stride + gi], pts[4 * stride + gi],
                                 pts[5 * stride + gi], eps, cosa);
        }
        S4_STAT(stats, 24 * KIND + (k == 64 ? 11 : 12), 1);
        S4_STAT(stats, 24 * KIND + 13, __popcll(r & (k >= 64 ? ~0ULL : ((1ULL << k) - 1ULL))));
        if (on && ((r >> lane) & 1ULL)) {
            atomicAdd(&sh.cntb[wv][slot], 1);
            if (MASK) atomicOr(&sh.maskb[wv][slot], 1ULL << (e2 & 63u));
        }
        qbh = (qbh + k) & 127;
        qbn -= k;
    };
// ... 179 lines not shown
        const int tot = __popcll(b0) + 2 * __popcll(b1) + 4 * __popcll(b2) + 8 * __popcll(b3);
        S4_STAT(stats, 24 * KIND + 1 + (h < 3 ? h : 3), 1);
        S4_STAT(stats, 24 * KIND + 5, __popcll(WB(ci < nk)));
        S4_STAT(stats, 24 * KIND + 7, tot);
        if (tot == 0) { S4_STAT(stats, 24 * KIND + 6, 1); continue; }
        int base = 0;
        if (lane == 0) base = atomicAdd(&sh.npairs, tot);
        base = __builtin_amdgcn_readfirstlane(base);
        auto mb = [&](uint64_t m) { return __builtin_amdgcn_mbcnt_hi((uint32_t)(m >> 32), __builtin_amdgcn_mbcnt_lo((uint32_t)m, 0)); };
        int pos = base + mb(b0) + 2 * mb(b1) + 4 * mb(b2) + 8 * mb(b3);
#pragma unroll
        for (int g = 0; g < S4_TG; g++) {
            const bool on = (surv >> g) & 1u;
            sh.plist[on ? pos : R * 64 * S4_TG] = (uint16_t)(((ci - (lo << 6)) << S4_GB) | g);
            pos += on ? 1 : 0;
        }
    }
    __syncthreads();
    const int npairs = sh.npairs;
    for (;;) {
        int bt = 0;
        if (lane == 0) bt = atomicAdd(&sh.next_batch, 1);
        bt = __builtin_amdgcn_readfirstlane(bt);
        if (bt * 64 >= npairs) break;
        score4_batch<KIND, R, MASK, F32, LIST>(sh, wv, lane, bt * 64, min(64, npairs - bt * 64), lo << 6, pts, stride, g0 * 64, K.prep, K.cls, K.orig,
                                         K.eps, K.cosa, counts, weird, masks, occ, mstride, g0, stats);
    }
}

template <class SH>
static __device__ __forceinline__ void s4_stage(SH &sh, const double *__restrict__ pts, int64_t stride, int64_t s,
                                                const uint64_t *__restrict__ enabled_words, const int64_t p0, const float *__restrict__ gb32,
                                                const uint32_t *__restrict__ gm32, const int64_t ngroups)
{
    static_assert(S4_TG % S4_W == 0, "every wave stages S4_TG / S4_W groups");
    const int tid = threadIdx.x, lane = tid & 63;
    const int wv = __builtin_amdgcn_readfirstlane(tid >> 6);
    constexpr int GPW = S4_TG / S4_W;
    double x[GPW], y[GPW], z[GPW], nx[GPW], ny[GPW], nz[GPW];
#pragma unroll
    for (int q = 0; q < GPW; q++) {
        const int64_t gi = p0 + (int64_t)(wv + q * S4_W) * 64 + lane;
        x[q] = pts[gi]; y[q] = pts[stride + gi]; z[q] = pts[2 * stride + gi];
        nx[q] = pts[3 * stride + gi]; ny[q] = pts[4 * stride + gi]; nz[q] = pts[5 * stride + gi];
    }
#pragma unroll
    for (int q = 0; q < GPW; q++) {
        const int g = wv + q * S4_W;
        const int64_t gi = p0 + (int64_t)g * 64 + lane;
        uint64_t v = valid_mask((gi >> 6) << 6, s);
        if (enabled_words != nullptr && v != 0) v &= enabled_words[gi >> 6];
        const bool on = (v >> (gi & 63)) & 1ULL;
        rh_f32x4 a = { 0.f, 0.f, 0.f, 0.f };
        rh_f32x2 b = { 0.f, 0.f };
        bool bad = false;
        if (on) {
            a.x = (float)x[q]; a.y = (float)y[q]; a.z = (float)z[q]; a.w = (float)nx[q]; b.x = (float)ny[q]; b.y = (float)nz[q];
            const float sum = (fabsf(a.x) + fabsf(a.y)) + (fabsf(a.z) + fabsf(a.w)) + (fabsf(b.x) + fabsf(b.y));
            bad = !(sum < __builtin_inff());
        }
        sh.pa[g][lane] = a;
        sh.pb[g][lane] = b;
        const uint64_t wb = WB(bad);
        if (lane == 0) { sh.weirdw[g] = wb != 0 ? 1 : 0; sh.len[g] = v; }
    }
    if (tid == 0) { sh.npairs = 0; sh.next_batch = 0; }
    if (tid < 2 * S4_TG) {
        const int64_t g = p0 / 64 + (tid >> 1);
        sh.gbox[tid >> 1][tid & 1] = ((const rh_f32x4 *)gb32)[(g < ngroups ? g : ngroups - 1) * 2 + (tid & 1)];
    }
    if (tid >= 64 && tid < 64 + S4_TG) {
        const int64_t g = p0 / 64 + (tid - 64);
        rh_u32x4 m = { 0xffffffffu, 0xffffffffu, 0xffffffffu, 0u };
        if (gm32 != nullptr) m = ((const rh_u32x4 *)gm32)[g < ngroups ? g : ngroups - 1];
        sh.gmask[tid - 64] = m;
    }
}

template <int R, bool MASK, bool F32, bool TAIL = false, bool LIST = false>
#ifndef RH_S4_MINBLK
#define RH_S4_MINBLK 7
#endif
__global__ void __launch_bounds__(64 * S4_W, (F32 && !(LIST && R == 16)) ? 8 : RH_S4_MINBLK)
score4_kernel(const double *__restrict__ pts, int64_t stride, int64_t s, const S4AllArgs A, int32_t *__restrict__ counts, int dbg_arg)
{
#ifdef RH_DIAG
    const int dbg = dbg_arg;
#else
    constexpr int dbg = 0;
    (void)dbg_arg;
#endif
    __shared__ S4Shared<R, MASK, LIST> sh;
    int64_t tile = blockIdx.x;
    int rowy = (int)blockIdx.y;
    if (!TAIL && A.rows > 0) {
        const int64_t k = blockIdx.x >> 3;
        rowy = (int)(k % A.rows);
        tile = ((k / A.rows) << 3) + (blockIdx.x & 7);
    }
    if (tile >= A.ntiles) return;
    if (A.stop != nullptr && *A.stop != 0) return;
    const int64_t g0 = tile * S4_TG;
    S4_STAT(A.stats, 96 + 0, 1);
    static_assert(!(TAIL && LIST), "the row-walking launch takes its candidates in bin order");
    int nch[4], total = 0;
    const int64_t st4 = LIST ? (tile / (S4_STG / S4_TG)) * 4 : 0;
#pragma unroll
    for (int k = 0; k < 4; k++) { nch[k] = ((LIST ? A.stcount[st4 + k] : *A.k[k].nk) + 63) >> 6; total += nch[k]; }
    bool ran = false, weird = false;
    unsigned live = 0;
    const uint64_t *staged_en = nullptr;
    (void)staged_en;
#define RH_S4_BODY(K)                                                                                                  \
    {                                                                                                                  \
        const int slo = max(lo, base) - base, shi = min(hi, base + nch[K]) - base;                                     \
        if (slo < shi) {                                                                                               \
            if (ran) __syncthreads();           \
            if (!ran || A.k[K].en != staged_en) {                                                                      \
                s4_stage(sh, pts, stride, s, A.k[K].en, g0 * 64, A.gb32, A.gm32, A.ngroups);                                   \
                staged_en = A.k[K].en;                                                                                 \
                S4_STAT(A.stats, 96 + 1, 1);                                                                           \
            } else { S4_STAT(A.stats, 96 + 2, 1); if (threadIdx.x == 0) { sh.npairs = 0; sh.next_batch = 0; } }      \
            __syncthreads();                                                                                           \
            live = 0;                                                                                                  \
            for (int g = 0; g < S4_TG; g++) live |= sh.len[g] != 0 ? (1u << g) : 0u;                                   \
            live = __builtin_amdgcn_readfirstlane(live);                                                               \
            { int ww = 0; for (int g = 0; g < S4_TG; g++) ww |= sh.weirdw[g]; weird = __builtin_amdgcn_readfirstlane(ww) != 0; }  \
            if (live != 0) score4_segment<K, R, MASK, F32, LIST>(sh, A.k[K], LIST ? A.stcount + (st4 + K) : A.k[K].nk, LIST ? A.stlist + (st4 + K) * A.stcap : nullptr, A.bstride, slo, shi, pts, stride, g0, live, weird, counts, dbg, A.masks, A.occ, A.mstride, A.stats); \
            else S4_STAT(A.stats, 96 + 3, 1);                                                                         \
            ran = true;                                                                                                \
        }                                                                                                              \
        base += nch[K];                                                                                                \
    }
    if (!TAIL) {
        const int lo = rowy * R, hi = min(total, lo + R);
        if (lo >= hi) return;
        int base = 0;
        RH_S4_BODY(RH_CONE)
        RH_S4_BODY(RH_CYLINDER)
        RH_S4_BODY(RH_SPHERE)
        RH_S4_BODY(RH_PLANE)
    } else {
        for (int lo = (A.row0 + (int)blockIdx.y) * R; lo < total; lo += (int)gridDim.y * R) {
            const int hi = min(total, lo + R);
            int base = 0;
            RH_S4_BODY(RH_CONE)
            RH_S4_BODY(RH_CYLINDER)
            RH_S4_BODY(RH_SPHERE)
            RH_S4_BODY(RH_PLANE)
        }
    }
#undef RH_S4_BODY
}

#ifdef RH_DIAG
struct S4AuditCand { rh_prep P; rh_cls C; double cNhi, wN, eDlo, wD, cosa, eps; int kind, usable; };

__global__ void __launch_bounds__(256)
cls_audit_kernel(const double *__restrict__ pts, int64_t stride, int64_t s, const S4AuditCand *__restrict__ cands, int ncand,
                 unsigned long long *__restrict__ out)
{
    const int64_t i = (int64_t)blockIdx.x * blockDim.x + threadIdx.x;
    const int c = blockIdx.y;
    if (c >= ncand) return;
    const S4AuditCand &Q = cands[c];
    double ea = 0.0, eb = 0.0;
    bool counted = false;
    if (i < s && Q.usable) {
        const double x = pts[i], y = pts[stride + i], z = pts[2 * stride + i];
        const double nx = pts[3 * stride + i], ny = pts[4 * stride + i], nz = pts[5 * stride + i];
        const rh_prep &P = Q.P;
        float a32, b32;
        double a64, b64;
        if (Q.kind == RH_PLANE) {
            cls_plane_ab(Q.C, (float)x, (float)y, (float)z, (float)nx, (float)ny, (float)nz, a32, b32);
            const double dn = (P.f[3] * nx + P.f[4] * ny) + P.f[5] * nz;
            const double d = (P.f[6] * (x - P.f[0]) + P.f[7] * (y - P.f[1])) + P.f[8] * (z - P.f[2]);
            a64 = (Q.cNhi - dn) / Q.wN;
            b64 = (fabs(d) - Q.eDlo) / Q.wD;
            ea = fabs((double)a32 - a64);
            eb = fabs((double)b32 - b64);
            counted = true;
        } else if (Q.kind == RH_SPHERE || Q.kind == RH_CYLINDER) {
            double qx, qy, qz, R, sgn;
            if (Q.kind == RH_SPHERE) {
                cls_round_ab<RH_SPHERE>(Q.C, (float)x, (float)y, (float)z, (float)nx, (float)ny, (float)nz, a32, b32);
                qx = x - P.f[0]; qy = y - P.f[1]; qz = z - P.f[2]; R = P.f[3]; sgn = P.f[4];
            } else {
                cls_round_ab<RH_CYLINDER>(Q.C, (float)x, (float)y, (float)z, (float)nx, (float)ny, (float)nz, a32, b32);
                const double tx = x - P.f[3], ty = y - P.f[4], tz = z - P.f[5];
                const double sd = (P.f[0] * tx + P.f[1] * ty) + P.f[2] * tz;
                qx = (x - P.f[0] * sd) - P.f[3]; qy = (y - P.f[1] * sd) - P.f[4]; qz = (z - P.f[2] * sd) - P.f[5];
                R = P.f[6]; sgn = P.f[7];
            }
            const double m2 = Q.cNhi, W2 = Q.wN, mv = Q.eDlo, Wv = Q.wD;
            const double n2 = (qx * qx + qy * qy) + qz * qz;
            const double qn = (qx * nx + qy * ny) + qz * nz;
            a64 = (fabs(n2 - (R * R + Q.eps * Q.eps)) - (2.0 * R * Q.eps - m2)) / W2;
            b64 = (mv + (Q.cosa * Q.cosa * n2 - sgn * qn * fabs(qn))) / Wv;
            if (a64 < 2.0) { ea = fabs((double)a32 - a64); eb = fabs((double)b32 - b64); }
            counted = true;
        } else if (Q.kind == RH_CONE) {
            bool near_axis;
            cls_cone_ab(Q.C, (float)x, (float)y, (float)z, (float)nx, (float)ny, (float)nz, a32, b32, near_axis);
            if (!near_axis) {
                double dist, dt;
                cone_frame(P, x, y, z, nx, ny, nz, dist, dt);
                const double an = sqrt((P.f[3] * P.f[3] + P.f[4] * P.f[4]) + P.f[5] * P.f[5]);
                const double wx = x - P.f[0], wy = y - P.f[1], wz = z - P.f[2];
                const double h = ((P.f[3] * wx + P.f[4] * wy) + P.f[5] * wz) / an;
                const double qx = wx - h * (P.f[3] / an), qy = wy - h * (P.f[4] / an), qz = wz - h * (P.f[5] / an);
// ... 14 lines not shown
    int cnt = counted ? 1 : 0;
    for (int off = 32; off > 0; off >>= 1) {
        const unsigned long long va = __shfl_down(ua, off), vb = __shfl_down(ub, off);
        ua = va > ua ? va : ua;
        ub = vb > ub ? vb : ub;
        cnt += __shfl_down(cnt, off);
    }
    if ((threadIdx.x & 63) == 0) { sa[threadIdx.x >> 6] = ua; sb[threadIdx.x >> 6] = ub; sc[threadIdx.x >> 6] = cnt; }
    __syncthreads();
    if (threadIdx.x == 0 && Q.kind >= 0 && Q.kind < 4) {
        unsigned long long ma = 0, mb = 0;
        int n = 0;
        for (int w = 0; w < 4; w++) { ma = sa[w] > ma ? sa[w] : ma; mb = sb[w] > mb ? sb[w] : mb; n += sc[w]; }
        atomicMax(&out[Q.kind * 2], ma);
        atomicMax(&out[Q.kind * 2 + 1], mb);
        atomicAdd(&out[8 + Q.kind], (unsigned long long)n);
    }
}

struct S4SoundCand { rh_prep P; rh_prepf Pf; rh_cls C; float box[RH_BOX_FIELDS]; int kind; int pad; };
struct S4SoundArgs { double eps[4], cosa[4]; int f32; };

template <int KIND>
static __device__ __forceinline__ void sound_one(const S4SoundCand &Q, const S4SoundArgs &A, double x, double y, double z, double nx, double ny,
                                                 double nz, const uint64_t valid, const rh_box32 &G, const rh_box32 &GS, const rh_box32 &GT, const rh_u32x4 gm, const rh_u32x4 sm, const int lane, unsigned long long *__restrict__ out)
{
    const double eps = A.eps[KIND], cosa = A.cosa[KIND];
    uint64_t ex;
    if (A.f32) ex = test_point<KIND>(Q.Pf, (float)x, (float)y, (float)z, (float)nx, (float)ny, (float)nz, eps, cosa);
    else ex = test_point<KIND>(Q.P, x, y, z, nx, ny, nz, eps, cosa);
    ex &= valid;
    const bool skip = box_skip32<KIND>(Q.box, G);
    const bool stskip = box_skip32<KIND>(Q.box, GS);
    const bool tlskip = box_skip32<KIND>(Q.box, GT);
    const bool exact_only = is_nan_bits(Q.C.f[RH_CLS_FLAG]);
    const float fx = (float)x, fy = (float)y, fz = (float)z, fnx = (float)nx, fny = (float)ny, fnz = (float)nz;
    float t, t0;
    if (KIND == RH_PLANE) { t = cls_plane_u(Q.C, fx, fy, fz, fnx, fny, fnz); t0 = cls_plane_u(Q.C, 0.f, 0.f, 0.f, 0.f, 0.f, 0.f); }
    else if (KIND == RH_CONE) { t = cls_cone_u(Q.C, fx, fy, fz, fnx, fny, fnz); t0 = 0.5f; }
    else { t = cls_round_u<KIND == RH_SPHERE ? RH_SPHERE : RH_CYLINDER>(Q.C, fx, fy, fz, fnx, fny, fnz);
           t0 = cls_round_u<KIND == RH_SPHERE ? RH_SPHERE : RH_CYLINDER>(Q.C, 0.f, 0.f, 0.f, 0.f, 0.f, 0.f); }
    const float sum = (fabsf(fx) + fabsf(fy)) + (fabsf(fz) + fabsf(fnx)) + (fabsf(fny) + fabsf(fnz));
    const bool weird = WB(!(sum < __builtin_inff()) && ((valid >> lane) & 1ULL)) != 0;
    const bool decided = !exact_only && !weird;
    const uint64_t sin_ = WB(decided && cls_sure(t)) & valid;
    const uint64_t amb = (WB(!decided || (KIND == RH_CONE ? (!cls_sure(t) && cls_sure(t - 1.0f)) : cls_undecided(t)))) & valid;
    const uint64_t sout = valid & ~sin_ & ~amb;
    float du, dn;
    bool near_axis = false;
    if (KIND == RH_PLANE) cls_plane_ab(Q.C, fx, fy, fz, fnx, fny, fnz, dn, du);
    else if (KIND == RH_CONE) cls_cone_ab(Q.C, fx, fy, fz, fnx, fny, fnz, du, dn, near_axis);
    else cls_round_ab<KIND == RH_SPHERE ? RH_SPHERE : RH_CYLINDER>(Q.C, fx, fy, fz, fnx, fny, fnz, du, dn);
    const uint64_t band = WB(!decided || near_axis || !(du > 1.0f)) & valid;
    if (lane == 0) {
        if (band != 0) atomicAdd(&out[40 + KIND], 1ULL);
        if (ex != 0) atomicAdd(&out[44 + KIND], 1ULL);
        if (stskip) atomicAdd(&out[48 + KIND], 1ULL);
        if (stskip && ex != 0) atomicAdd(&out[52 + KIND], 1ULL);
        if (tlskip) atomicAdd(&out[56 + KIND], 1ULL);
        if (tlskip && ex != 0) atomicAdd(&out[60 + KIND], 1ULL);
        if (KIND == RH_PLANE) {
            const bool gskip = !nsig_meet(Q.box, gm), sskip = !nsig_meet(Q.box, sm);
            if (gskip) atomicAdd(&out[64], 1ULL);
            if (gskip && ex != 0) atomicAdd(&out[65], 1ULL);
            if (sskip) atomicAdd(&out[66], 1ULL);
            if (sskip && ex != 0) atomicAdd(&out[67], 1ULL);
        }
        unsigned long long *o = out + KIND * 10;
        atomicAdd(&o[0], 1ULL);
        if (skip) atomicAdd(&o[1], 1ULL);
        if (skip && ex != 0) atomicAdd(&o[2], 1ULL);
        atomicAdd(&o[3], (unsigned long long)__popcll(valid));
        if (sin_) atomicAdd(&o[4], (unsigned long long)__popcll(sin_));
        if (sout) atomicAdd(&o[5], (unsigned long long)__popcll(sout));
        if (sin_ & ~ex) atomicAdd(&o[6], (unsigned long long)__popcll(sin_ & ~ex));
        if (sout & ex) atomicAdd(&o[7], (unsigned long long)__popcll(sout & ex));
        if (ex) atomicAdd(&o[8], (unsigned long long)__popcll(ex));
        if (blockIdx.x == 0 && !exact_only && cls_sure(t0)) atomicAdd(&o[9], 1ULL);
    }
}

__global__ void __launch_bounds__(64)
cls_sound_kernel(const double *__restrict__ pts, int64_t stride, int64_t s, const float *__restrict__ gb32, const float *__restrict__ st32, const float *__restrict__ tile32, const uint32_t *__restrict__ gm32, const uint32_t *__restrict__ stm32, const S4SoundCand *__restrict__ cands,
                 int ncand, const S4SoundArgs A, unsigned long long *__restrict__ out)
{
    const int lane = threadIdx.x;
    const int64_t g = blockIdx.x;
    const int64_t i = g * 64 + lane;
    const uint64_t valid = valid_mask(g * 64, s);
    const bool on = (valid >> lane) & 1ULL;
    const double x = on ? pts[i] : 0.0, y = on ? pts[stride + i] : 0.0, z = on ? pts[2 * stride + i] : 0.0;
    const double nx = on ? pts[3 * stride + i] : 0.0, ny = on ? pts[4 * stride + i] : 0.0, nz = on ? pts[5 * stride + i] : 0.0;
    rh_box32 G;
    G.cx = gb32[g * 8 + 0]; G.cy = gb32[g * 8 + 1]; G.cz = gb32[g * 8 + 2]; G.hx = gb32[g * 8 + 3];
    G.hy = gb32[g * 8 + 4]; G.hz = gb32[g * 8 + 5]; G.hr = gb32[g * 8 + 6];
    rh_box32 GS;
    {
        const float *b = st32 + (g / S4_STG) * 8;
        GS.cx = b[0]; GS.cy = b[1]; GS.cz = b[2]; GS.hx = b[3]; GS.hy = b[4]; GS.hz = b[5]; GS.hr = b[6];
    }
    rh_box32 GT;
    {
        const float *b = tile32 + (g / S4_TG) * 8;
        GT.cx = b[0]; GT.cy = b[1]; GT.cz = b[2]; GT.hx = b[3]; GT.hy = b[4]; GT.hz = b[5]; GT.hr = b[6];
    }
    const rh_u32x4 gm = ((const rh_u32x4 *)gm32)[g], sm = ((const rh_u32x4 *)stm32)[g / S4_STG];
    for (int c = blockIdx.y; c < ncand; c += gridDim.y) {
        const S4SoundCand &Q = cands[c];
        switch (Q.kind) {
        case RH_PLANE: sound_one<RH_PLANE>(Q, A, x, y, z, nx, ny, nz, valid, G, GS, GT, gm, sm, lane, out); break;
        case RH_SPHERE: sound_one<RH_SPHERE>(Q, A, x, y, z, nx, ny, nz, valid, G, GS, GT, gm, sm, lane, out); break;
        case RH_CYLINDER: sound_one<RH_CYLINDER>(Q, A, x, y, z, nx, ny, nz, valid, G, GS, GT, gm, sm, lane, out); break;
        case RH_CONE: sound_one<RH_CONE>(Q, A, x, y, z, nx, ny, nz, valid, G, GS, GT, gm, sm, lane, out); break;
        default: break;
        }
    }
}

__global__ void __launch_bounds__(256)
cls_cone_dbg_kernel(const rh_cls C, const float *__restrict__ pts, int64_t n, float *__restrict__ ua, float *__restrict__ ub,
                    uint8_t *__restrict__ near_out)
{
    const int64_t i = (int64_t)blockIdx.x * blockDim.x + threadIdx.x;
    if (i >= n) return;
    float a, b;
    bool near_axis;
    cls_cone_ab(C, pts[i], pts[n + i], pts[2 * n + i], pts[3 * n + i], pts[4 * n + i], pts[5 * n + i], a, b, near_axis);
    ua[i] = a;
    ub[i] = b;
    near_out[i] = near_axis ? 1 : 0;
}

#endif

#ifndef RH_UNP_BLOCK
#define RH_UNP_BLOCK 512
#endif
#ifndef RH_UNP_MULTI
#define RH_UNP_MULTI 3072
#endif
constexpr int S4_UNP_WORDS = 8192, S4_UNP_WORDS_MULTI = RH_UNP_MULTI;
constexpr int S6_UNROLL = 4;

template <bool WAVEWORD, int BLK = 512>
__global__ void __launch_bounds__(BLK)
unpermute6_kernel(const rh_u64x2 *__restrict__ ent, const int32_t *__restrict__ cursor, int64_t mstride, const int32_t *__restrict__ perm,
                  int64_t swords, int64_t seg_words, const uint64_t *__restrict__ segmask, int64_t smstride, uint64_t *__restrict__ out)
{
    extern __shared__ unsigned long long seg[];
    __shared__ uint32_t ring[BLK / 64][128];
    const int lane = threadIdx.x & 63, wv = threadIdx.x >> 6;
    const int64_t row = blockIdx.x;
    const int64_t w0 = (int64_t)blockIdx.y * seg_words;
    const int nw = (int)(swords - w0 < seg_words ? swords - w0 : seg_words);
    for (int t = threadIdx.x; t < nw; t += BLK) seg[t] = 0ULL;
    const int n = min(cursor[row], (int32_t)mstride);
    __syncthreads();
    const int32_t lo = (int32_t)(w0 << 6), span = nw << 6;
    const rh_u64x2 *__restrict__ src = ent + row * mstride;
    const uint64_t *__restrict__ sm = segmask != nullptr ? segmask + (int64_t)blockIdx.y * smstride : nullptr;
    if (WAVEWORD) {
        for (int i0 = wv * 4; i0 < n; i0 += (BLK / 64) * 4) {
            rh_u64x2 e[4];
            int32_t j[4];
#pragma unroll
            for (int k = 0; k < 4; k++) {
                e[k] = src[min(i0 + k, n - 1)];
                j[k] = perm[((int64_t)e[k].x << 6) + lane] - lo;
            }
#pragma unroll
            for (int k = 0; k < 4; k++)
                if (i0 + k < n && ((e[k].y >> lane) & 1ULL) && j[k] >= 0 && j[k] < span) atomicOr(&seg[j[k] >> 6], 1ULL << (j[k] & 63));
        }
        __syncthreads();
        uint64_t *__restrict__ dstw = out + row * swords + w0;
        for (int t = threadIdx.x; t < nw; t += BLK) dstw[t] = seg[t];
        return;
    }
    int head = 0, fill = 0;
    auto drain = [&](int k) {
        wave_lds_sync();
        if (lane < k) {
            const uint32_t e = ring[wv][(head + lane) & 127];
            const int32_t j = perm[e] - lo;
            if (j >= 0 && j < span) atomicOr(&seg[j >> 6], 1ULL << (j & 63));
        }
        head = (head + k) & 127;
        fill -= k;
    };
    for (int i0 = threadIdx.x; i0 - lane < n; i0 += BLK * S6_UNROLL) {
        rh_u64x2 e[S6_UNROLL];
// ... 52 lines not shown

__global__ void gb32_kernel(const double *__restrict__ gb, int64_t gstride, int64_t ngroups, float *__restrict__ out)
{
    const int64_t g = (int64_t)blockIdx.x * blockDim.x + threadIdx.x;
    if (g >= ngroups) return;
    const double c[3] = { gb[g], gb[gstride + g], gb[2 * gstride + g] };
    const double h[3] = { gb[3 * gstride + g], gb[4 * gstride + g], gb[5 * gstride + g] };
    float o[8];
    box_to_f32(c, h, o);
#pragma unroll
    for (int k = 0; k < 8; k++) out[g * 8 + k] = o[k];
}

__global__ void st32_kernel(const double *__restrict__ gb, int64_t gstride, int64_t ngroups, int k_groups, int64_t nst, float *__restrict__ out)
{
    const int64_t st = (int64_t)blockIdx.x * blockDim.x + threadIdx.x;
    if (st >= nst) return;
    double lo[3] = { __builtin_inf(), __builtin_inf(), __builtin_inf() }, hi[3] = { -__builtin_inf(), -__builtin_inf(), -__builtin_inf() };
    bool bad = false;
    for (int64_t g = st * k_groups; g < (st + 1) * k_groups && g < ngroups; g++)
#pragma unroll
        for (int k = 0; k < 3; k++) {
            const double cc = gb[k * gstride + g], hh = gb[(3 + k) * gstride + g];
            bad |= !(fabs(cc) < __builtin_inf()) || !(fabs(hh) < __builtin_inf());
            lo[k] = fmin(lo[k], cc - hh);
            hi[k] = fmax(hi[k], cc + hh);
        }
    double c3[3], h3[3];
#pragma unroll
    for (int k = 0; k < 3; k++) {
        c3[k] = 0.5 * lo[k] + 0.5 * hi[k];
        h3[k] = fmax(hi[k] - c3[k], c3[k] - lo[k]) * 1.000000000001 + (fabs(lo[k]) + fabs(hi[k])) * 1e-15;
        bad |= !(fabs(c3[k]) < __builtin_inf()) || !(h3[k] < __builtin_inf());
    }
    float o[8];
    box_to_f32(c3, h3, o);
#pragma unroll
    for (int k = 0; k < 8; k++) out[st * 8 + k] = bad ? __builtin_nanf("") : o[k];
}

__global__ void __launch_bounds__(256)
nsig_kernel(const double *__restrict__ pts, int64_t stride, int64_t s, int64_t ngroups, uint32_t *__restrict__ out, unsigned long long *__restrict__ maxlen)
{
    __shared__ uint32_t m[4][4];
    const int lane = threadIdx.x & 63, wv = threadIdx.x >> 6;
    const int64_t g = (int64_t)blockIdx.x * 4 + wv;
    if (lane < 4) m[wv][lane] = 0u;
    __syncthreads();
    const int64_t i = g * 64 + lane;
    double len = 0.0;
    if (g < ngroups && i < s) {
        const double nx = pts[3 * stride + i], ny = pts[4 * stride + i], nz = pts[5 * stride + i];
        uint32_t w[3];
        nsig_point_bits(nx, ny, nz, w);
        if (w[0] != 0u) atomicOr(&m[wv][0], w[0]);
        if (w[1] != 0u) atomicOr(&m[wv][1], w[1]);
        if (w[2] != 0u) atomicOr(&m[wv][2], w[2]);
        const double l = sqrt((nx * nx + ny * ny) + nz * nz);
        if (l < __builtin_inf()) len = l;
    }
    unsigned long long lb = __builtin_bit_cast(unsigned long long, len);
    for (int off = 32; off > 0; off >>= 1) { const unsigned long long v = __shfl_down(lb, off); lb = v > lb ? v : lb; }
    if (lane == 0 && lb != 0ULL) atomicMax(maxlen, lb);
    __syncthreads();
    if (g < ngroups && lane < 4) out[g * 4 + lane] = m[wv][lane];
}

__global__ void nsig_st_kernel(const uint32_t *__restrict__ gm, int64_t ngroups, int k_groups, int64_t nst, uint32_t *__restrict__ out)
{
    const int64_t st = (int64_t)blockIdx.x * blockDim.x + threadIdx.x;
    if (st >= nst) return;
    uint32_t w[4] = { 0u, 0u, 0u, 0u };
    for (int64_t g = st * k_groups; g < (st + 1) * k_groups && g < ngroups; g++)
#pragma unroll
        for (int k = 0; k < 3; k++) w[k] |= gm[g * 4 + k];
#pragma unroll
    for (int k = 0; k < 4; k++) out[st * 4 + k] = w[k];
}

struct StCullArgs {
    const float *box[4];
    const int32_t *nk[4];
    int64_t bstride, stcap;
    const float *st32;
    const uint32_t *stm32;
    uint16_t *stlist;
    int32_t *stcount;
};

template <int KIND>
static __device__ __forceinline__ void st_cull_kind(const StCullArgs &A, const int64_t st)
{
    constexpr int Q = 4;
    __shared__ int32_t wsum[2][Q * 4];
    const int tid = threadIdx.x, lane = tid & 63, wv = tid >> 6;
    const int nk = *A.nk[KIND];
    int32_t *cnt = A.stcount + st * 4 + KIND;
    if (nk <= 0) { if (tid == 0) *cnt = 0; return; }
    rh_box32 G;
    {
        const float *b = A.st32 + st * 8;
        G.cx = b[0]; G.cy = b[1]; G.cz = b[2]; G.hx = b[3]; G.hy = b[4]; G.hz = b[5]; G.hr = b[6];
    }
    rh_u32x4 GM = { 0xffffffffu, 0xffffffffu, 0xffffffffu, 0u };
    if (KIND == RH_PLANE && A.stm32 != nullptr) GM = ((const rh_u32x4 *)A.stm32)[st];
    uint16_t *__restrict__ list = A.stlist + (st * 4 + KIND) * A.stcap;
    constexpr int NB = S4Fields<KIND>::NBOX;
    const float *__restrict__ box = A.box[KIND];
    int base = 0, it = 0;
    for (int j0 = 0; j0 < nk; j0 += Q * 256, it++) {
        float B[Q][RH_BOX_FIELDS];
#pragma unroll
        for (int q = 0; q < Q; q++) {
            const int cand = j0 + q * 256 + tid, cl = cand < nk ? cand : 0;
#pragma unroll
            for (int f = 0; f < NB; f++) B[q][f] = box[(int64_t)f * A.bstride + cl];
        }
        uint64_t m[Q];
        bool keep[Q];
#pragma unroll
        for (int q = 0; q < Q; q++) {
            keep[q] = j0 + q * 256 + tid < nk && !box_skip32<KIND>(B[q], G);
            if (KIND == RH_PLANE) keep[q] = keep[q] && nsig_meet(B[q], GM);
            m[q] = WB(keep[q]);
            if (lane == 0) wsum[it & 1][q * 4 + wv] = __popcll(m[q]);
        }
        __syncthreads();
        int run = base;
#pragma unroll
        for (int q = 0; q < Q; q++) {
            int off = run;
#pragma unroll
            for (int w = 0; w < 4; w++) { const int v = wsum[it & 1][q * 4 + w]; off += w < wv ? v : 0; run += v; }
            if (keep[q]) list[off + __builtin_amdgcn_mbcnt_hi((uint32_t)(m[q] >> 32), __builtin_amdgcn_mbcnt_lo((uint32_t)m[q], 0))] = (uint16_t)(j0 + q * 256 + tid);
        }
        base = run;
    }
    if (tid == 0) *cnt = base;
}

__global__ void __launch_bounds__(256)
st_cull_kernel(const StCullArgs A)
{
    const int64_t st = blockIdx.x;
    switch (blockIdx.y) {
    case RH_PLANE: st_cull_kind<RH_PLANE>(A, st); break;
    case RH_SPHERE: st_cull_kind<RH_SPHERE>(A, st); break;
    case RH_CYLINDER: st_cull_kind<RH_CYLINDER>(A, st); break;
    default: st_cull_kind<RH_CONE>(A, st); break;
    }
}

inline int cdiv4(int64_t a, int64_t b) { return (int)((a + b - 1) / b); }

}

int rhk_gb32_build(rh_cloud *c)
{
    if (c->ngroups == 0 || c->gb32 == nullptr) return RH_OK;
    hipLaunchKernelGGL(gb32_kernel, dim3(cdiv4(c->ngroups, 256)), dim3(256), 0, c->stream, c->gb, c->ng_pad, c->ngroups, c->gb32);
    if (c->st32 != nullptr && c->nst > 0)
        hipLaunchKernelGGL(st32_kernel, dim3(cdiv4(c->nst, 64)), dim3(64), 0, c->stream, c->gb, c->ng_pad, c->ngroups, S4_STG, c->nst, c->st32);
    if (c->tile32 != nullptr && c->ntile > 0)
        hipLaunchKernelGGL(st32_kernel, dim3(cdiv4(c->ntile, 64)), dim3(64), 0, c->stream, c->gb, c->ng_pad, c->ngroups, S4_TG, c->ntile, c->tile32);
    RH_HIP(hipGetLastError());
    c->nrm_len = 0.0;
    if (c->gm32 != nullptr && c->stm32 != nullptr && c->s > 0) {
        rh_dev<unsigned long long> d_len;
        RH_TRY(d_len.alloc(1));
        RH_HIP(hipMemsetAsync(d_len, 0, sizeof(unsigned long long), c->stream));
        hipLaunchKernelGGL(nsig_kernel, dim3(cdiv4(c->ngroups, 4)), dim3(256), 0, c->stream, c->sub, c->s_pad, c->s, c->ngroups, c->gm32, d_len);
        hipLaunchKernelGGL(nsig_st_kernel, dim3(cdiv4(c->nst, 64)), dim3(64), 0, c->stream, c->gm32, c->ngroups, S4_STG, c->nst, c->stm32);
        RH_HIP(hipGetLastError());
        unsigned long long h_len = 0;
        RH_HIP(hipMemcpyAsync(&h_len, d_len, sizeof h_len, hipMemcpyDeviceToHost, c->stream));
        RH_HIP(hipStreamSynchronize(c->stream));
        c->nrm_len = __builtin_bit_cast(double, h_len);
    }
    return RH_OK;
}

static inline int64_t stlist_bytes(const rh_cloud *c, int64_t cap) { return (int64_t)sizeof(uint16_t) * c->nst * 4 * cap; }
static int ensure_stlists(rh_cloud *c, rh_batch_ws &w, int64_t cap)
{
    if (w.d_stlist != nullptr && cap <= w.stlist_cap && w.stlist_nst == c->nst) return RH_OK;
    const int64_t ncap = std::max<int64_t>(cap, 1024);
    w.stlist_cap = 0;
    RH_TRY(w.d_stcount.grow(c->stream, c->nst * 4));
    RH_TRY(w.d_stlist.grow(c->stream, c->nst * 4 * ncap));
    w.stlist_cap = ncap;
    w.stlist_nst = c->nst;
    return RH_OK;
}

int rhk_score4_all(rh_cloud *c, rh_batch_ws &w, const rh_score_job &job, int32_t *launch_info)
{
    const rh_bins &B = job.bins;
    const int32_t nk_total_bound = job.bound;
    int32_t *const d_counts = job.d_counts;
    uint64_t *const d_masks_int = job.d_masks_int;
    const bool open_count = job.open_count;
    const bool f32cloud = c->f32;
    const bool on_subset = job.points.pts == nullptr;
    const rh_s4_points PS = on_subset ? rh_s4_points{ c->sub, c->s_pad, c->s, c->ngroups, c->gb32 } : job.points;
    const int64_t ntiles = (PS.ngroups + S4_TG - 1) / S4_TG;
    const int nchunks = cdiv4(nk_total_bound, 64) + 3;
    if (ntiles == 0 || nk_total_bound <= 0) return RH_OK;
    if (B.cls[0] == nullptr || B.box[0] == nullptr || !rh_score_v4_enabled(c) || PS.gb32 == nullptr || (d_masks_int != nullptr && !w.masks4)) {
        rh_set_error("internal: the culled score kernel without its records (classifier, culling, group boxes, mask lists)");
        return RH_E_INTERNAL;
    }
    const int dbg = (int)rh_opt_int(c, RH_OPT_G2_DBG, 0);
    S4AllArgs A;
    for (int k = 0; k < 4; k++)
        A.k[k] = { (const rh_cls *)B.cls[k], B.box[k], B.prep[k], B.orig[k], job.nk[k], job.en[k], job.eps[k], job.cosa[k] };
    A.stop = job.stop;
    A.ntiles = ntiles;
    A.bstride = job.bstride;
    A.ngroups = PS.ngroups;
    A.gb32 = PS.gb32;
    const bool nsig_on = on_subset && c->gm32 != nullptr && rh_opt_int(c, RH_OPT_NSIG, 0) != 2;
    A.gm32 = nsig_on ? (const uint32_t *)c->gm32 : nullptr;
    A.masks = d_masks_int;
    A.occ = d_masks_int ? w.d_occ : nullptr;
    A.mstride = d_masks_int ? w.mstride4 : 0;
    A.stats = nullptr;
#ifdef RH_DIAG
    A.stats = c->s4_stats;
#endif
    A.stlist = nullptr; A.stcount = nullptr; A.stcap = 0;
    const int64_t st_opt = rh_opt_int(c, RH_OPT_ST_CULL, 0);
    bool use_lists = !open_count && on_subset && dbg == 0 && c->st32 != nullptr && c->nst >= 2 && nk_total_bound <= 16384 && st_opt != 2;
    if (use_lists && st_opt == 0)
        use_lists = nk_total_bound >= 1024 && ntiles >= (rh_opt_int(c, RH_OPT_BATCHES_IN_FLIGHT, 1) > 1 ? 1000 : 3000);
    const int64_t lcap = std::max<int64_t>(((int64_t)nk_total_bound + 63) / 64 * 64, 1024);
    if (use_lists) {
        const int64_t mb = rh_opt_int(c, RH_OPT_ST_LIST_MB, 0);
        const int64_t need = stlist_bytes(c, lcap);
        if (need > ((mb > 0 ? mb : 512) << 20) || (w.stlist_nomem > 0 && need >= w.stlist_nomem)) use_lists = false;
    }
    if (use_lists) {
        const int rc = ensure_stlists(c, w, lcap);
        if (rc == RH_E_NOMEM) {
            (void)hipGetLastError();
            rh_set_error("%s", "");
            w.stlist_nomem = stlist_bytes(c, lcap);
            use_lists = false;
        } else if (rc != RH_OK) return rc;
    }
    if (use_lists) {
        StCullArgs SA;
        for (int k = 0; k < 4; k++) { SA.box[k] = B.box[k]; SA.nk[k] = job.nk[k]; }
        SA.bstride = job.bstride; SA.stcap = w.stlist_cap; SA.st32 = c->st32; SA.stm32 = nsig_on && c->stm32 != nullptr ? (const uint32_t *)c->stm32 : nullptr; SA.stlist = w.d_stlist; SA.stcount = w.d_stcount;
        hipLaunchKernelGGL(st_cull_kernel, dim3((unsigned)c->nst, 4), dim3(256), 0, c->stream, SA);
        A.stlist = w.d_stlist; A.stcount = w.d_stcount; A.stcap = w.stlist_cap;
        if (job.ev_listed != nullptr) RH_HIP(hipEventRecord(job.ev_listed, c->stream));
    }
    const int env_r = (int)rh_opt_int(c, RH_OPT_S4_ROWS, 0);
    int R;
    if (env_r == 4 || env_r == 8 || ((env_r == 1 || env_r == 2 || env_r == 12 || env_r == 16) && !open_count)) R = env_r;
    else if (open_count) R = ntiles * ((nchunks + 7) / 8) < 3000 ? 4 : 8;
    else if (ntiles * ((nchunks + 15) / 16) >= 16384) R = 16;
    else if (ntiles * ((nchunks + 11) / 12) >= 3000) R = use_lists ? 16 : 12;
    else if (ntiles * ((nchunks + 3) / 4) >= 4000) R = 4;
    else R = 2;
    int64_t rows = (nchunks + R - 1) / R;
    if (!open_count && launch_info != nullptr) { launch_info[0] = R; launch_info[1] = use_lists ? 1 : 0; launch_info[2] = (int32_t)rows; launch_info[3] = (int32_t)ntiles; }
    if (rows > 65535) { rh_set_error("batch of %d candidates is too large for one launch", nk_total_bound); return RH_E_INVALID; }
    const bool pad8 = ntiles >= 1024;
    dim3 grid((unsigned)(pad8 ? ((ntiles + 7) / 8) * 8 : ntiles), (unsigned)rows);
    const unsigned tiles_x = grid.x;
    A.row0 = 0;
    A.rows = 0;
#ifndef RH_S4_XROW_MAX
#define RH_S4_XROW_MAX 4096
#endif
    if (rows > 1 && ((ntiles + 7) / 8) * 8 * rows <= RH_S4_XROW_MAX) {
        A.rows = (int)rows;
        grid = dim3((unsigned)(((ntiles + 7) / 8) * 8 * rows), 1);
    }
    const int loop_max = open_count ? 32 : 0;
    auto launch_tail = [&](unsigned ny) {
        const dim3 gt(tiles_x, ny);
        if (f32cloud) {
            if (R == 4) hipLaunchKernelGGL((score4_kernel<4, false, true, true>), gt, dim3(64 * S4_W), 0, c->stream, PS.pts, PS.stride, PS.s, A, d_counts, dbg);
            else hipLaunchKernelGGL((score4_kernel<8, false, true, true>), gt, dim3(64 * S4_W), 0, c->stream, PS.pts, PS.stride, PS.s, A, d_counts, dbg);
        } else {
            if (R == 4) hipLaunchKernelGGL((score4_kernel<4, false, false, true>), gt, dim3(64 * S4_W), 0, c->stream, PS.pts, PS.stride, PS.s, A, d_counts, dbg);
            else hipLaunchKernelGGL((score4_kernel<8, false, false, true>), gt, dim3(64 * S4_W), 0, c->stream, PS.pts, PS.stride, PS.s, A, d_counts, dbg);
        }
    };
    if (loop_max > 0 && d_masks_int == nullptr && nchunks <= loop_max) {
        launch_tail(1);
        RH_HIP(hipGetLastError());
        return RH_OK;
    }
#define RH_S4_LAUNCH(RR, MM, FF)                                                                                                              \
    do {                                                                                                                                      \
        if (use_lists) hipLaunchKernelGGL((score4_kernel<RR, MM, FF, false, true>), grid, dim3(64 * S4_W), 0, c->stream, PS.pts, PS.stride, PS.s, A, d_counts, dbg); \
        else hipLaunchKernelGGL((score4_kernel<RR, MM, FF>), grid, dim3(64 * S4_W), 0, c->stream, PS.pts, PS.stride, PS.s, A, d_counts, dbg);  \
    } while (0)
#define RH_S4_LAUNCH_R(MM, FF)                                                                                         \
    do {                                                                                                               \
        if (R == 4) RH_S4_LAUNCH(4, MM, FF);                                                                           \
        else if (R == 1) RH_S4_LAUNCH(1, MM, FF);                                                                      \
        else if (R == 2) RH_S4_LAUNCH(2, MM, FF);                                                                      \
        else if (R == 12) RH_S4_LAUNCH(12, MM, FF);                                                                    \
        else if (R == 16) RH_S4_LAUNCH(16, MM, FF);                                                                    \
        else RH_S4_LAUNCH(8, MM, FF);                                                                                  \
    } while (0)
    if (f32cloud) {
        if (d_masks_int != nullptr) RH_S4_LAUNCH_R(true, true); else RH_S4_LAUNCH_R(false, true);
    } else if (d_masks_int != nullptr) RH_S4_LAUNCH_R(true, false);
    else RH_S4_LAUNCH_R(false, false);
#undef RH_S4_LAUNCH_R
#undef RH_S4_LAUNCH
    if (open_count) {
        if (d_masks_int != nullptr) { rh_set_error("rhk_score4_all: masks need an exact candidate count"); return RH_E_INTERNAL; }
        A.row0 = (int)rows;
        launch_tail(2);
    }
    RH_HIP(hipGetLastError());
    return RH_OK;
}

namespace {
__global__ void __launch_bounds__(256)
store_cls_kernel(const rh_prep *p0, const rh_prep *p1, const rh_prep *p2, const rh_prep *p3, int32_t n0, int32_t n1, int32_t n2, int32_t n3,
                 int32_t b1, int32_t b2, int32_t b3, int32_t total, double e0, double e1, double e2, double e3, double c0, double c1, double c2,
                 double c3, double M, double Nm, double Ln, rh_cls *__restrict__ cls, float *__restrict__ box, int64_t bstride)
{
    const int32_t g = blockIdx.x * blockDim.x + threadIdx.x;
    if (g >= total) return;
    const int q = (g >= b1 ? 1 : 0) + (g >= b2 ? 1 : 0) + (g >= b3 ? 1 : 0);
    const int32_t slot = g - (q == 0 ? 0 : (q == 1 ? b1 : (q == 2 ? b2 : b3)));
    const int32_t n = q == 0 ? n0 : (q == 1 ? n1 : (q == 2 ? n2 : n3));
    if (slot >= n) return;
    const rh_prep *pp = q == 0 ? p0 : (q == 1 ? p1 : (q == 2 ? p2 : p3));
    const double eps = q == 0 ? e0 : (q == 1 ? e1 : (q == 2 ? e2 : e3)), cosa = q == 0 ? c0 : (q == 1 ? c1 : (q == 2 ? c2 : c3));
    const rh_prep P = pp[slot];
    cls_make(P, q, eps, cosa, M, Nm, cls[g], box + g, bstride, nullptr, false, Ln);
}
}

int rhk_store_cls(rh_cloud *c, const rh_prep *const prep[4], const int32_t n[4], const int32_t pbase[5], const double eps[4],
                  const double cosa[4], void *d_cls, float *d_box, int64_t bstride)
{
    if (pbase[4] <= 0) return RH_OK;
    hipLaunchKernelGGL(store_cls_kernel, dim3((unsigned)cdiv4(pbase[4], 256)), dim3(256), 0, c->stream, prep[0], prep[1], prep[2], prep[3], n[0], n[1],
                       n[2], n[3], pbase[1], pbase[2], pbase[3], pbase[4], eps[0], eps[1], eps[2], eps[3], cosa[0], cosa[1], cosa[2], cosa[3],
                       c->coord_mag, c->nrm_mag, c->nrm_len, (rh_cls *)d_cls, d_box, bstride);
    RH_HIP(hipGetLastError());
    return RH_OK;
}

int rhk_score4_dis(rh_cloud *c, int64_t first, int64_t cnt, rh_score_job job)
{
    if (cnt <= 0 || job.bound <= 0) return RH_OK;
    const int64_t ng = (cnt + 63) / 64;
    if (ng > c->ng_pad) { rh_set_error("rhk_score4_dis: %lld groups", (long long)ng); return RH_E_INTERNAL; }
    RH_TRY(rhk_group_bounds_of(c, c->dis + first, c->dis_stride, cnt, ng, c->dis_gb, c->ng_pad));
    hipLaunchKernelGGL(gb32_kernel, dim3(cdiv4(ng, 256)), dim3(256), 0, c->stream, c->dis_gb, c->ng_pad, ng, c->dis_gb32);
    RH_HIP(hipGetLastError());
    job.points = { c->dis + first, c->dis_stride, cnt, ng, c->dis_gb32 };
    return rhk_score4_all(c, c->ws[0], job);
}

#ifdef RH_DIAG
extern "C" int rh_dbg_cls_audit(rh_cloud *c, const rh_shape *shapes, int32_t b, const rh_params *p, double *out)
{
    if (c == nullptr || out == nullptr || p == nullptr || b < 0 || (b > 0 && shapes == nullptr)) { rh_set_error("rh_dbg_cls_audit: bad arguments"); return RH_E_INVALID; }
    for (int i = 0; i < 12; i++) out[i] = 0.0;
    if (b == 0 || c->s == 0) return RH_OK;
    RH_HIP(hipSetDevice(c->device));
    std::vector<S4AuditCand> h((size_t)b);
    for (int32_t i = 0; i < b; i++) {
        S4AuditCand &Q = h[(size_t)i];
        Q.kind = shapes[i].kind;
        Q.usable = 0;
        if (Q.kind < 0 || Q.kind > 3) continue;
        rh_prep_host(shapes[i], &Q.P);
        double d4[4] = { 0, 0, 0, 0 };
        cls_make(Q.P, Q.kind, p->eps[Q.kind], p->cos_alpha[Q.kind], c->coord_mag, c->nrm_mag, Q.C, nullptr, 0, d4, c->f32);
        Q.cNhi = d4[0]; Q.wN = d4[1]; Q.eDlo = d4[2]; Q.wD = d4[3]; Q.cosa = p->cos_alpha[Q.kind]; Q.eps = p->eps[Q.kind];
        Q.usable = !(Q.C.f[RH_CLS_FLAG] != Q.C.f[RH_CLS_FLAG]) && Q.wN > 0 && Q.wD > 0;
    }
    rh_dev<S4AuditCand> d_c;
    rh_dev<unsigned long long> d_o;
    RH_TRY(d_c.alloc(b));
    RH_TRY(d_o.alloc(12));
    RH_HIP(hipMemcpyAsync(d_c, h.data(), sizeof(S4AuditCand) * (size_t)b, hipMemcpyHostToDevice, c->stream));
    RH_HIP(hipMemsetAsync(d_o, 0, sizeof(unsigned long long) * 12, c->stream));
    for (int32_t c0 = 0; c0 < b; c0 += 32768) {
        const int32_t nb = std::min<int32_t>(32768, b - c0);
        hipLaunchKernelGGL(cls_audit_kernel, dim3((unsigned)cdiv4(c->s, 256), (unsigned)nb), dim3(256), 0, c->stream, c->sub, c->s_pad,
                           c->s, d_c + c0, nb, d_o);
    }
    unsigned long long ho[12];
    RH_HIP(hipMemcpyAsync(ho, d_o, sizeof ho, hipMemcpyDeviceToHost, c->stream));
    RH_HIP(hipStreamSynchronize(c->stream));
    for (int i = 0; i < 8; i++) out[i] = __builtin_bit_cast(double, ho[i]);
    for (int i = 8; i < 12; i++) out[i] = (double)ho[i];
    return RH_OK;
}

static int cls_soundness_run(rh_cloud *c, const rh_shape *shapes, int32_t b, const rh_params *p, uint64_t *out, const int first, const int nout)
{
    if (c == nullptr || out == nullptr || p == nullptr || b < 0 || (b > 0 && shapes == nullptr)) { rh_set_error("rh_dbg_cls_soundness: bad arguments"); return RH_E_INVALID; }
    for (int i = 0; i < nout; i++) out[i] = 0;
    if (b == 0 || c->s == 0 || c->ngroups == 0 || c->gb32 == nullptr || c->st32 == nullptr || c->tile32 == nullptr || c->gm32 == nullptr || c->stm32 == nullptr) return RH_OK;
    RH_HIP(hipSetDevice(c->device));
    std::vector<S4SoundCand> h((size_t)b);
    for (int32_t i = 0; i < b; i++) {
        S4SoundCand &Q = h[(size_t)i];
        Q.kind = shapes[i].kind;
        Q.pad = 0;
        if (Q.kind < 0 || Q.kind > 3) { Q.kind = -1; continue; }
        rh_prep_host(shapes[i], &Q.P);
        Q.Pf = prepf_of_kind(Q.P, Q.kind);
        cls_make(Q.P, Q.kind, p->eps[Q.kind], p->cos_alpha[Q.kind], c->coord_mag, c->nrm_mag, Q.C, Q.box, 1, nullptr, c->f32, c->nrm_len);
    }
    S4SoundArgs A;
    for (int k = 0; k < 4; k++) { A.eps[k] = p->eps[k]; A.cosa[k] = p->cos_alpha[k]; }
    A.f32 = c->f32 ? 1 : 0;
    rh_dev<S4SoundCand> d_c;
    rh_dev<unsigned long long> d_o;
    RH_TRY(d_c.alloc(b));
    RH_TRY(d_o.alloc(72));
    RH_HIP(hipMemcpyAsync(d_c, h.data(), sizeof(S4SoundCand) * (size_t)b, hipMemcpyHostToDevice, c->stream));
    RH_HIP(hipMemsetAsync(d_o, 0, sizeof(unsigned long long) * 72, c->stream));
    hipLaunchKernelGGL(cls_sound_kernel, dim3((unsigned)c->ngroups, (unsigned)std::min<int32_t>(b, 64)), dim3(64), 0, c->stream, c->sub, c->s_pad, c->s,
                       c->gb32, c->st32, c->tile32, c->gm32, c->stm32, d_c, b, A, d_o);
    unsigned long long ho[72];
    RH_HIP(hipMemcpyAsync(ho, d_o, sizeof ho, hipMemcpyDeviceToHost, c->stream));
    RH_HIP(hipStreamSynchronize(c->stream));
    for (int i = 0; i < nout; i++) out[i] = (uint64_t)ho[first + i];
    return RH_OK;
}

extern "C" int rh_dbg_cls_soundness(rh_cloud *c, const rh_shape *shapes, int32_t b, const rh_params *p, uint64_t *out)
{
    return cls_soundness_run(c, shapes, b, p, out, 0, 56);
}

extern "C" int rh_dbg_cls_soundness_tiles(rh_cloud *c, const rh_shape *shapes, int32_t b, const rh_params *p, uint64_t *out)
{
    return cls_soundness_run(c, shapes, b, p, out, 56, 8);
}

extern "C" int rh_dbg_cls_soundness_nsig(rh_cloud *c, const rh_shape *shapes, int32_t b, const rh_params *p, uint64_t *out)
{
    return cls_soundness_run(c, shapes, b, p, out, 64, 4);
}

extern "C" int rh_dbg_nsig(const rh_shape *shape, const rh_params *p, double M, double Nm, double Ln, int f32, uint32_t *mask_out,
                           const double *dirs, int64_t ndirs, int32_t *cells_out)
{
    if (p == nullptr || ndirs < 0 || (ndirs > 0 && (dirs == nullptr || cells_out == nullptr)) || (shape != nullptr && mask_out == nullptr)) {
        rh_set_error("rh_dbg_nsig: bad arguments");
        return RH_E_INVALID;
    }
    if (shape != nullptr) {
        if (shape->kind != RH_PLANE) { rh_set_error("rh_dbg_nsig: planes only"); return RH_E_INVALID; }
        rh_prep P;
        rh_prep_host(*shape, &P);
        rh_cls C;
        float box[RH_BOX_FIELDS];
        cls_make(P, RH_PLANE, p->eps[RH_PLANE], p->cos_alpha[RH_PLANE], M, Nm, C, box, 1, nullptr, f32 != 0, Ln);
        for (int k = 0; k < 3; k++) mask_out[k] = __builtin_bit_cast(uint32_t, box[5 + k]);
    }
    for (int64_t i = 0; i < ndirs; i++) {
        uint32_t w[3];
        nsig_point_bits(dirs[3 * i], dirs[3 * i + 1], dirs[3 * i + 2], w);
        if ((w[0] & w[1] & w[2]) == 0xffffffffu) cells_out[i] = -2;
        else if ((w[0] | w[1] | w[2]) == 0u) cells_out[i] = -1;
        else cells_out[i] = nsig_cell(dirs[3 * i], dirs[3 * i + 1], dirs[3 * i + 2]);
    }
    return RH_OK;
}

extern "C" int rh_dbg_group_boxes(rh_cloud *c, double *out, int64_t cap, int64_t *ngroups_out)
{
    if (c == nullptr || ngroups_out == nullptr || cap < 0) { rh_set_error("rh_dbg_group_boxes: bad arguments"); return RH_E_INVALID; }
    *ngroups_out = c->gb == nullptr ? 0 : c->ngroups;
    if (out == nullptr || cap < *ngroups_out || *ngroups_out == 0) return RH_OK;
    RH_HIP(hipSetDevice(c->device));
    std::vector<double> h((size_t)c->ngroups * 6);
    const double *gb = c->gb;
    for (int k = 0; k < 6; k++)
        RH_HIP(hipMemcpyAsync(h.data() + (size_t)k * c->ngroups, gb + (int64_t)k * c->ng_pad, sizeof(double) * (size_t)c->ngroups, hipMemcpyDeviceToHost, c->stream));
    RH_HIP(hipStreamSynchronize(c->stream));
    for (int64_t g = 0; g < c->ngroups; g++)
        for (int k = 0; k < 6; k++) out[6 * g + k] = h[(size_t)k * c->ngroups + g];
    return RH_OK;
}

extern "C" int rh_dbg_cylbox(const rh_shape *shape, const rh_params *p, double M, double Nm, int f32, const double *boxes, int64_t n,
                             uint8_t *skip_out, uint8_t *ball_out, float *fields_out)
{
    if (shape == nullptr || p == nullptr || n < 0 || (n > 0 && (boxes == nullptr || skip_out == nullptr || ball_out == nullptr))) {
        rh_set_error("rh_dbg_cylbox: bad arguments");
        return RH_E_INVALID;
    }
    if (shape->kind != RH_CYLINDER) { rh_set_error("rh_dbg_cylbox: cylinders only"); return RH_E_INVALID; }
    rh_prep P;
    rh_prep_host(*shape, &P);
    rh_cls C;
    float box[RH_BOX_FIELDS];
    cls_make(P, RH_CYLINDER, p->eps[RH_CYLINDER], p->cos_alpha[RH_CYLINDER], M, Nm, C, box, 1, nullptr, f32 != 0);
    if (fields_out != nullptr)
        for (int k = 0; k < RH_BOX_FIELDS; k++) fields_out[k] = box[k];
    for (int64_t i = 0; i < n; i++) {
        float o[8];
        box_to_f32(boxes + 6 * i, boxes + 6 * i + 3, o);
        rh_box32 G;
// ... 207 lines not shown
```

Baseline: 82.38 million candidates/s.

## Add plane-specific point ordering with separate group boxes for plane scoring

Builds a second permutation of the subset, using a per-block kd split on normals of up to 1024 points, so that groups of 64 points have tight normal ranges. Plane candidates are then scored against this reordered copy with its own group and supertile boxes, nsig masks and enabled bits. The aim is to let plane candidates cull more groups through the normal-angle test. The cost is a second 6×s copy of the subset in memory, extra build work at cloud creation, and an enabled-bit remap kernel on every enabled update. It is on by default when the tile count reaches 256.

```diff
diff --git a/include/ransac_hip.h b/include/ransac_hip.h
--- a/include/ransac_hip.h
+++ b/include/ransac_hip.h
@@ -7,7 +7,7 @@
 extern "C" {
 #endif
 
-#define RH_VERSION 121
+#define RH_VERSION 122
 
 enum {
     RH_OK = 0,
diff --git a/include/ransac_hip_diag.h b/include/ransac_hip_diag.h
--- a/include/ransac_hip_diag.h
+++ b/include/ransac_hip_diag.h
@@ -14,6 +14,8 @@
 int rh_dbg_nsig(const rh_shape *shape, const rh_params *p, double M, double Nm, double Ln, int f32, uint32_t *mask_out ,
                 const double *dirs, int64_t ndirs, int32_t *cells_out);
 int rh_dbg_group_boxes(rh_cloud *c, double *out, int64_t cap, int64_t *ngroups_out);
+int rh_dbg_plane_order(rh_cloud *c, int64_t *info_out , double *sub_out, double *pl_out, int32_t *src_out, float *gb32_out,
+                       uint32_t *gm32_out, uint64_t *en_out);
 int rh_dbg_cylbox(const rh_shape *shape, const rh_params *p, double M, double Nm, int f32, const double *boxes, int64_t n,
                   uint8_t *skip_out, uint8_t *ball_out, float *fields_out );
 int rh_dbg_cls_round(const rh_shape *shape, const rh_params *p, double M, double Nm, int f32, int64_t n, const double *xyz,
diff --git a/ransac.jl_amd/_lib.py b/ransac.jl_amd/_lib.py
--- a/ransac.jl_amd/_lib.py
+++ b/ransac.jl_amd/_lib.py
@@ -268,6 +268,7 @@
     "rh_dbg_cls_soundness_nsig": (C.c_int, [_vp, _sp, C.c_int32, _pp, C.POINTER(C.c_uint64)]),
     "rh_dbg_nsig": (C.c_int, [_sp, _pp, C.c_double, C.c_double, C.c_double, C.c_int, C.POINTER(C.c_uint32), _dp, C.c_int64, _i32p]),
     "rh_dbg_group_boxes": (C.c_int, [_vp, _dp, C.c_int64, C.POINTER(C.c_int64)]),
+    "rh_dbg_plane_order": (C.c_int, [_vp, _i64p, _dp, _dp, _i32p, C.POINTER(C.c_float), C.POINTER(C.c_uint32), _u64p]),
     "rh_dbg_cylbox": (C.c_int, [_sp, _pp, C.c_double, C.c_double, C.c_int, _dp, C.c_int64, C.POINTER(C.c_uint8), C.POINTER(C.c_uint8), C.POINTER(C.c_float)]),
     "rh_dbg_cls_round": (C.c_int, [_sp, _pp, C.c_double, C.c_double, C.c_int, C.c_int64, _dp, _dp, C.POINTER(C.c_float), C.POINTER(C.c_float),
                                    C.POINTER(C.c_float), _dp]),
@@ -326,7 +327,11 @@
         if which == "diag":
             sigs.update(DIAG_SIGNATURES)
         for name, (res, args) in sigs.items():
-            f = getattr(L, name)
+            f = getattr(L, name, None)
+            if f is None and os.environ.get("RH_LIB_PATH"):
+                continue
+            if f is None:
+                raise AttributeError("%s does not export %s" % (path, name))
             f.restype = res
             f.argtypes = args
         if L.rh_build_variant() != (1 if which == "diag" else 0):
diff --git a/ransac.jl_amd/csrc/cloud.hip b/ransac.jl_amd/csrc/cloud.hip
--- a/ransac.jl_amd/csrc/cloud.hip
+++ b/ransac.jl_amd/csrc/cloud.hip
@@ -482,6 +482,8 @@
         }
     }
     stamp("subset order, gather, boxes");
+    if (n > 0 && s > 0) CK(rhk_plane_order_build(c));
+    stamp("plane order");
     CK(rhk_enabled_replace(c, nullptr));
     CKH(hipStreamSynchronize(c->stream));
     stamp("enabled bits");
diff --git a/ransac.jl_amd/csrc/enabled.hip b/ransac.jl_amd/csrc/enabled.hip
--- a/ransac.jl_amd/csrc/enabled.hip
+++ b/ransac.jl_amd/csrc/enabled.hip
@@ -330,7 +330,7 @@
                        c->enabled, c->sub_idx0, c->s, c->swords, c->sub_enabled, reset_list ? 1 : 0, c->sub, c->s_pad,
                        c->dis, c->dis_stride, c->d_ndis);
     RH_HIP(hipGetLastError());
-    return RH_OK;
+    return rhk_plane_enabled_sync(c);
 }
 
 static int read_ndis(rh_cloud *c)
diff --git a/ransac.jl_amd/csrc/kdorder.hip b/ransac.jl_amd/csrc/kdorder.hip
--- a/ransac.jl_amd/csrc/kdorder.hip
+++ b/ransac.jl_amd/csrc/kdorder.hip
@@ -6,6 +6,9 @@
 #include <hipcub/hipcub.hpp>
 
 #include "rh_internal.h"
+#ifdef RH_DIAG
+#include "ransac_hip_diag.h"
+#endif
 
 namespace {
 
@@ -141,6 +144,115 @@
 }
 
 struct KdNode { int32_t lo, hi; };
+
+constexpr int PO_ST = 1024;
+constexpr int PO_THREADS = 512;
+
+__global__ void __launch_bounds__(PO_THREADS)
+plane_order_kernel(const double *__restrict__ sub, int64_t stride, const int32_t *__restrict__ blk_lo, int32_t *__restrict__ src)
+{
+    __shared__ float nv[3][PO_ST];
+    __shared__ uint64_t key[PO_ST];
+    __shared__ uint16_t ord[PO_ST];
+    __shared__ uint32_t box[16][6];
+    __shared__ int nlo[2][18];
+    __shared__ int nnode[2];
+    const int tid = threadIdx.x;
+    const int64_t base = blk_lo[blockIdx.x];
+    const int cnt = (int)(blk_lo[blockIdx.x + 1] - base);
+    for (int i = tid; i < PO_ST; i += PO_THREADS) {
+        const bool in = i < cnt;
+#pragma unroll
+        for (int k = 0; k < 3; k++) nv[k][i] = in ? (float)sub[(3 + k) * stride + base + i] : 0.0f;
+        ord[i] = (uint16_t)i;
+    }
+    if (tid == 0) { nlo[0][0] = 0; nlo[0][1] = cnt; nnode[0] = 1; }
+    __syncthreads();
+    for (int level = 0; level < 4; level++) {
+        const int *lo = nlo[level & 1];
+        const int nn = nnode[level & 1];
+        for (int t = tid; t < 16 * 6; t += PO_THREADS) box[t / 6][t % 6] = (t % 6) < 3 ? 0xffffffffu : 0u;
+        __syncthreads();
+        auto node_of = [&](int i) { int nd = 0; for (int k = 1; k < nn; k++) nd += lo[k] <= i ? 1 : 0; return nd; };
+        for (int i = tid; i < cnt; i += PO_THREADS) {
+            const int nd = node_of(i);
+            if (lo[nd + 1] - lo[nd] <= 64) continue;
+            const int j = ord[i];
+#pragma unroll
+            for (int k = 0; k < 3; k++) {
+                const float v = nv[k][j];
+                if (v - v == 0.0f) { atomicMin(&box[nd][k], ord32(v)); atomicMax(&box[nd][3 + k], ord32(v)); }
+            }
+        }
+        __syncthreads();
+        for (int i = tid; i < PO_ST; i += PO_THREADS) {
+            const int j = ord[i];
+            int nd = 31;
+            uint32_t sk = (uint32_t)i;
+            if (i < cnt) {
+                nd = node_of(i);
+                if (lo[nd + 1] - lo[nd] > 64) {
+                    int ax = 0;
+                    float best = -2.0f;
+#pragma unroll
+                    for (int k = 0; k < 3; k++) {
+                        const uint32_t bl = box[nd][k], bh = box[nd][3 + k];
+                        const float e = bl <= bh ? unord32(bh) - unord32(bl) : -1.0f;
+                        if (e > best) { best = e; ax = k; }
+                    }
+                    sk = ord32(nv[ax][j]);
+                }
+            }
+            key[i] = ((uint64_t)nd << 42) | ((uint64_t)sk << 10) | (uint64_t)j;
+        }
+        __syncthreads();
+        for (int k = 2; k <= PO_ST; k <<= 1)
+            for (int j = k >> 1; j > 0; j >>= 1) {
+                const int i = ((tid & ~(j - 1)) << 1) | (tid & (j - 1)), p = i | j;
+                const uint64_t a = key[i], b = key[p];
+                if ((a > b) == ((i & k) == 0)) { key[i] = b; key[p] = a; }
+                __syncthreads();
+            }
+        for (int i = tid; i < PO_ST; i += PO_THREADS) ord[i] = (uint16_t)(key[i] & 1023u);
+        if (tid == 0) {
+            int *nx = nlo[(level + 1) & 1];
+            int m = 0;
+            for (int q = 0; q < nn; q++) {
+                const int c0 = lo[q + 1] - lo[q];
+                nx[m++] = lo[q];
+                if (c0 > 64) nx[m++] = lo[q] + ((c0 / 64 + 1) / 2) * 64;
+            }
+            nx[m] = cnt;
+            nnode[(level + 1) & 1] = m;
+        }
+        __syncthreads();
+    }
+    for (int i = tid; i < cnt; i += PO_THREADS) src[base + i] = (int32_t)base + ord[i];
+}
+
+__global__ void __launch_bounds__(256)
+plane_gather_kernel(const double *__restrict__ sub, int64_t stride, int64_t s, const int32_t *__restrict__ src, double *__restrict__ out)
+{
+    const int64_t i = (int64_t)blockIdx.x * blockDim.x + threadIdx.x;
+    if (i >= s) return;
+    const int64_t j = src[i];
+#pragma unroll
+    for (int k = 0; k < 6; k++) out[k * stride + i] = sub[k * stride + j];
+}
+
+__global__ void __launch_bounds__(256)
+plane_enabled_kernel(const uint64_t *__restrict__ sub_enabled, int64_t s, int64_t swords, const int32_t *__restrict__ src,
+                     uint64_t *__restrict__ out)
+{
+    const int64_t i = (int64_t)blockIdx.x * blockDim.x + threadIdx.x;
+    bool bit = false;
+    if (i < s) {
+        const int64_t j = src[i];
+        bit = (sub_enabled[j >> 6] >> (j & 63)) & 1ULL;
+    }
+    const uint64_t w = __builtin_amdgcn_ballot_w64(bit);
+    if ((threadIdx.x & 63) == 0 && (i >> 6) < swords) out[i >> 6] = w;
+}
 
 __device__ __forceinline__ unsigned long long ord64(double v)
 {
@@ -293,3 +405,75 @@
     c->nrm_mag = __builtin_bit_cast(double, h_mags[1]);
     return RH_OK;
 }
+
+int rhk_plane_order_build(rh_cloud *c)
+{
+    if (!c->use_groups || c->s <= 0 || c->nst <= 0) return RH_OK;
+    if (c->s > (int64_t)0x7fffffff) { rh_set_error("rhk_plane_order_build: subset of %lld points", (long long)c->s); return RH_E_INVALID; }
+    std::vector<int32_t> lo;
+    {
+        std::vector<KdNode> stack(1, KdNode{ 0, (int32_t)c->s });
+        while (!stack.empty()) {
+            const KdNode nd = stack.back();
+            stack.pop_back();
+            const int32_t cnt = nd.hi - nd.lo;
+            if (cnt <= PO_ST) { lo.push_back(nd.lo); continue; }
+            const int32_t nl = ((cnt / 64 + 1) / 2) * 64;
+            stack.push_back(KdNode{ nd.lo + nl, nd.hi });
+            stack.push_back(KdNode{ nd.lo, nd.lo + nl });
+        }
+        lo.push_back((int32_t)c->s);
+    }
+    const int64_t nblk = (int64_t)lo.size() - 1;
+    rh_dev<int32_t> d_lo;
+    RH_TRY(d_lo.alloc((int64_t)lo.size()));
+    RH_HIP(hipMemcpyAsync(d_lo, lo.data(), sizeof(int32_t) * lo.size(), hipMemcpyHostToDevice, c->stream));
+    RH_TRY(c->pl_sub.alloc(6 * c->s_pad));
+    RH_TRY(c->pl_src.alloc(c->s_pad));
+    RH_TRY(c->pl_st32.alloc(8 * c->nst));
+    RH_TRY(c->pl_stm32.alloc(4 * c->nst));
+    RH_TRY(c->pl_gb32.alloc(8 * c->ng_pad));
+    RH_TRY(c->pl_gm32.alloc(4 * c->ng_pad));
+    RH_TRY(c->pl_enabled.alloc(c->swords));
+    RH_HIP(hipMemsetAsync(c->pl_sub, 0, sizeof(double) * 6 * (size_t)c->s_pad, c->stream));
+    RH_HIP(hipMemsetAsync(c->pl_src, 0, sizeof(int32_t) * (size_t)c->s_pad, c->stream));
+    hipLaunchKernelGGL(plane_order_kernel, dim3((unsigned)nblk), dim3(PO_THREADS), 0, c->stream, c->sub, c->s_pad, d_lo.get(), c->pl_src.get());
+    hipLaunchKernelGGL(plane_gather_kernel, dim3(cdivq(c->s, 256)), dim3(256), 0, c->stream, c->sub, c->s_pad, c->s, c->pl_src.get(), c->pl_sub.get());
+    RH_HIP(hipGetLastError());
+    return rhk_plane_boxes(c);
+}
+
+int rhk_plane_enabled_sync(rh_cloud *c)
+{
+    if (c->pl_enabled == nullptr || c->s <= 0) return RH_OK;
+    hipLaunchKernelGGL(plane_enabled_kernel, dim3(cdivq(c->swords * 64, 256)), dim3(256), 0, c->stream, c->sub_enabled, c->s, c->swords,
+                       c->pl_src.get(), c->pl_enabled.get());
+    RH_HIP(hipGetLastError());
+    return RH_OK;
+}
+
+#ifdef RH_DIAG
+extern "C" int rh_dbg_plane_order(rh_cloud *c, int64_t *info_out, double *sub_out, double *pl_out, int32_t *src_out, float *gb32_out,
+                                  uint32_t *gm32_out, uint64_t *en_out)
+{
+    if (c == nullptr || info_out == nullptr) { rh_set_error("rh_dbg_plane_order: bad arguments"); return RH_E_INVALID; }
+    const bool has = c->pl_sub != nullptr;
+    info_out[0] = c->s; info_out[1] = c->ngroups; info_out[2] = c->nst; info_out[3] = has ? 1 : 0;
+    if (!has || c->s <= 0) return RH_OK;
+    RH_HIP(hipSetDevice(c->device));
+    const size_t s = (size_t)c->s;
+    for (int k = 0; k < 6; k++) {
+        if (sub_out != nullptr) RH_HIP(hipMemcpyAsync(sub_out + k * s, c->sub + k * c->s_pad, sizeof(double) * s, hipMemcpyDeviceToHost, c->stream));
+        if (pl_out != nullptr) RH_HIP(hipMemcpyAsync(pl_out + k * s, c->pl_sub + k * c->s_pad, sizeof(double) * s, hipMemcpyDeviceToHost, c->stream));
+    }
+    if (src_out != nullptr) RH_HIP(hipMemcpyAsync(src_out, c->pl_src, sizeof(int32_t) * s, hipMemcpyDeviceToHost, c->stream));
+    if (gb32_out != nullptr) RH_HIP(hipMemcpyAsync(gb32_out, c->pl_gb32, sizeof(float) * 8 * (size_t)c->ngroups, hipMemcpyDeviceToHost, c->stream));
+    if (gm32_out != nullptr) RH_HIP(hipMemcpyAsync(gm32_out, c->pl_gm32, sizeof(uint32_t) * 4 * (size_t)c->ngroups, hipMemcpyDeviceToHost, c->stream));
+    if (en_out != nullptr) {
+        RH_HIP(hipMemcpyAsync(en_out, c->sub_enabled, sizeof(uint64_t) * (size_t)c->swords, hipMemcpyDeviceToHost, c->stream));
+        RH_HIP(hipMemcpyAsync(en_out + c->swords, c->pl_enabled, sizeof(uint64_t) * (size_t)c->swords, hipMemcpyDeviceToHost, c->stream));
+    }
+    RH_HIP(hipStreamSynchronize(c->stream));
+    return RH_OK;
+}
+#endif
diff --git a/ransac.jl_amd/csrc/options.cpp b/ransac.jl_amd/csrc/options.cpp
--- a/ransac.jl_amd/csrc/options.cpp
+++ b/ransac.jl_amd/csrc/options.cpp
@@ -31,6 +31,7 @@
     RH_O(RH_OPT_BATCHES_IN_FLIGHT, "batches_in_flight", "RH_BATCHES_IN_FLIGHT", T_INT),
     RH_O(RH_OPT_ST_LIST_MB, "st_list_mb", "RH_ST_LIST_MB", T_INT),
     RH_O(RH_OPT_NSIG, "nsig", "RH_NSIG", T_INT),
+    RH_O(RH_OPT_PLANE_ORDER, "plane_order", "RH_PLANE_ORDER", T_INT),
 #ifdef RH_DIAG
     RH_O(RH_OPT_CREATE_PROF, "create_prof", "RH_CREATE_PROF", T_FLAG),
     RH_O(RH_OPT_AABB_HOST, "aabb_host", "RH_AABB_HOST", T_FLAG),
@@ -142,6 +143,7 @@
         case RH_OPT_BATCHES_IN_FLIGHT: ok = value >= 0 && value <= RH_MAX_IN_FLIGHT; break;
         case RH_OPT_ST_LIST_MB: ok = value >= 0 && value <= (1 << 20); break;
         case RH_OPT_NSIG: ok = value == 0 || value == 2; break;
+        case RH_OPT_PLANE_ORDER: ok = value >= 0 && value <= 2; break;
         default: break;
         }
         if (!ok) { rh_set_error("rh_set_option: value %lld is not valid for '%s'", (long long)value, key); return RH_E_INVALID; }
diff --git a/ransac.jl_amd/csrc/rh_internal.h b/ransac.jl_amd/csrc/rh_internal.h
--- a/ransac.jl_amd/csrc/rh_internal.h
+++ b/ransac.jl_amd/csrc/rh_internal.h
@@ -38,6 +38,7 @@
     RH_OPT_BATCHES_IN_FLIGHT,
     RH_OPT_ST_LIST_MB,
     RH_OPT_NSIG,
+    RH_OPT_PLANE_ORDER,
     RH_OPT_N_PRODUCT,
     RH_OPT_CREATE_PROF = RH_OPT_N_PRODUCT, RH_OPT_AABB_HOST, RH_OPT_SUB_ORDER, RH_OPT_KD_HOST, RH_OPT_NO_SPREAD, RH_OPT_OCT_CHAIN_W,
     RH_OPT_NO_MANAGED_STORE, RH_OPT_OCT_ONE_WINDOW, RH_OPT_OCT_WINDOW_ITERS, RH_OPT_NO_FUSED_SCORE, RH_OPT_NO_PIPELINE,
@@ -252,6 +253,13 @@
     rh_dev<uint32_t> gm32;
     rh_dev<uint32_t> stm32;
     double nrm_len = 0;
+    rh_dev<double> pl_sub;
+    rh_dev<int32_t> pl_src;
+    rh_dev<float> pl_gb32;
+    rh_dev<uint32_t> pl_gm32;
+    rh_dev<float> pl_st32;
+    rh_dev<uint32_t> pl_stm32;
+    rh_dev<uint64_t> pl_enabled;
     rh_dev<double> dis_gb;
 
     rh_enabled_state en;
@@ -401,6 +409,9 @@
 int rhk_score4_dis(rh_cloud *c, int64_t first, int64_t cnt, rh_score_job job);
 int rhk_cloud_aabb(rh_cloud *c, const double *d_xyz, int64_t n, double lo[3], double hi[3], bool has[3], double *mag);
 int rhk_kd_order(rh_cloud *c, const double *d_xyz, const double *d_nrm, const int32_t *d_idx0);
+int rhk_plane_order_build(rh_cloud *c);
+int rhk_plane_enabled_sync(rh_cloud *c);
+int rhk_plane_boxes(rh_cloud *c);
 int rhk_score_kind_dis(rh_cloud *c, int kind, int64_t first, int64_t cnt, const rh_prep *d_prep, const int32_t *d_orig,
                        const int32_t *d_nk, int32_t nk_bound, double eps, double cosa, int32_t *d_counts);
 int rhk_group_bounds(rh_cloud *c);
diff --git a/ransac.jl_amd/csrc/score4.hip b/ransac.jl_amd/csrc/score4.hip
--- a/ransac.jl_amd/csrc/score4.hip
+++ b/ransac.jl_amd/csrc/score4.hip
@@ -56,6 +56,10 @@
     const int32_t *orig, *nk;
     const uint64_t *en;
     double eps, cosa;
+    const double *pts;
+    int64_t stride;
+    const float *gb32;
+    const uint32_t *gm32;
 };
 struct S4AllArgs {
     const int32_t *stop;
@@ -63,8 +67,6 @@
     int rows;
     S4KindArgs k[4];
     int64_t ntiles, bstride, ngroups;
-    const float *gb32;
-    const uint32_t *gm32;
     uint64_t *masks;
     uint8_t *occ;
     int64_t mstride;
@@ -410,7 +412,7 @@
 #define RH_S4_MINBLK 7
 #endif
 __global__ void __launch_bounds__(64 * S4_W, (F32 && !(LIST && R == 16)) ? 8 : RH_S4_MINBLK)
-score4_kernel(const double *__restrict__ pts, int64_t stride, int64_t s, const S4AllArgs A, int32_t *__restrict__ counts, int dbg_arg)
+score4_kernel(int64_t s, const S4AllArgs A, int32_t *__restrict__ counts, int dbg_arg)
 {
 #ifdef RH_DIAG
     const int dbg = dbg_arg;
@@ -438,15 +440,18 @@
     bool ran = false, weird = false;
     unsigned live = 0;
     const uint64_t *staged_en = nullptr;
+    const double *staged_pts = nullptr;
     (void)staged_en;
+    (void)staged_pts;
 #define RH_S4_BODY(K)                                                                                                  \
     {                                                                                                                  \
         const int slo = max(lo, base) - base, shi = min(hi, base + nch[K]) - base;                                     \
         if (slo < shi) {                                                                                               \
             if (ran) __syncthreads();           \
-            if (!ran || A.k[K].en != staged_en) {                                                                      \
-                s4_stage(sh, pts, stride, s, A.k[K].en, g0 * 64, A.gb32, A.gm32, A.ngroups);                                   \
+            if (!ran || A.k[K].en != staged_en || A.k[K].pts != staged_pts) {    \
+                s4_stage(sh, A.k[K].pts, A.k[K].stride, s, A.k[K].en, g0 * 64, A.k[K].gb32, A.k[K].gm32, A.ngroups);   \
                 staged_en = A.k[K].en;                                                                                 \
+                staged_pts = A.k[K].pts;                                                                               \
                 S4_STAT(A.stats, 96 + 1, 1);                                                                           \
             } else { S4_STAT(A.stats, 96 + 2, 1); if (threadIdx.x == 0) { sh.npairs = 0; sh.next_batch = 0; } }      \
             __syncthreads();                                                                                           \
@@ -454,7 +459,7 @@
             for (int g = 0; g < S4_TG; g++) live |= sh.len[g] != 0 ? (1u << g) : 0u;                                   \
             live = __builtin_amdgcn_readfirstlane(live);                                                               \
             { int ww = 0; for (int g = 0; g < S4_TG; g++) ww |= sh.weirdw[g]; weird = __builtin_amdgcn_readfirstlane(ww) != 0; }  \
-            if (live != 0) score4_segment<K, R, MASK, F32, LIST>(sh, A.k[K], LIST ? A.stcount + (st4 + K) : A.k[K].nk, LIST ? A.stlist + (st4 + K) * A.stcap : nullptr, A.bstride, slo, shi, pts, stride, g0, live, weird, counts, dbg, A.masks, A.occ, A.mstride, A.stats); \
+            if (live != 0) score4_segment<K, R, MASK, F32, LIST>(sh, A.k[K], LIST ? A.stcount + (st4 + K) : A.k[K].nk, LIST ? A.stlist + (st4 + K) * A.stcap : nullptr, A.bstride, slo, shi, A.k[K].pts, A.k[K].stride, g0, live, weird, counts, dbg, A.masks, A.occ, A.mstride, A.stats); \
             else S4_STAT(A.stats, 96 + 3, 1);                                                                         \
             ran = true;                                                                                                \
         }                                                                                                              \
@@ -635,7 +640,7 @@
 
 __global__ void __launch_bounds__(64)
 cls_sound_kernel(const double *__restrict__ pts, int64_t stride, int64_t s, const float *__restrict__ gb32, const float *__restrict__ st32, const float *__restrict__ tile32, const uint32_t *__restrict__ gm32, const uint32_t *__restrict__ stm32, const S4SoundCand *__restrict__ cands,
-                 int ncand, const S4SoundArgs A, unsigned long long *__restrict__ out)
+                 int ncand, const S4SoundArgs A, const int kinds, unsigned long long *__restrict__ out)
 {
     const int lane = threadIdx.x;
     const int64_t g = blockIdx.x;
@@ -660,6 +665,7 @@
     const rh_u32x4 gm = ((const rh_u32x4 *)gm32)[g], sm = ((const rh_u32x4 *)stm32)[g / S4_STG];
     for (int c = blockIdx.y; c < ncand; c += gridDim.y) {
         const S4SoundCand &Q = cands[c];
+        if (Q.kind < 0 || Q.kind > 3 || !((kinds >> Q.kind) & 1)) continue;
         switch (Q.kind) {
         case RH_PLANE: sound_one<RH_PLANE>(Q, A, x, y, z, nx, ny, nz, valid, G, GS, GT, gm, sm, lane, out); break;
         case RH_SPHERE: sound_one<RH_SPHERE>(Q, A, x, y, z, nx, ny, nz, valid, G, GS, GT, gm, sm, lane, out); break;
@@ -878,7 +884,7 @@
     const float *box[4];
     const int32_t *nk[4];
     int64_t bstride, stcap;
-    const float *st32;
+    const float *st32, *st32_plane;
     const uint32_t *stm32;
     uint16_t *stlist;
     int32_t *stcount;
@@ -895,7 +901,7 @@
     if (nk <= 0) { if (tid == 0) *cnt = 0; return; }
     rh_box32 G;
     {
-        const float *b = A.st32 + st * 8;
+        const float *b = (KIND == RH_PLANE ? A.st32_plane : A.st32) + st * 8;
         G.cx = b[0]; G.cy = b[1]; G.cz = b[2]; G.hx = b[3]; G.hy = b[4]; G.hz = b[5]; G.hr = b[6];
     }
     rh_u32x4 GM = { 0xffffffffu, 0xffffffffu, 0xffffffffu, 0u };
@@ -976,6 +982,37 @@
     return RH_OK;
 }
 
+int rhk_plane_boxes(rh_cloud *c)
+{
+    if (c->pl_sub == nullptr || c->ngroups == 0) return RH_OK;
+    rh_dev<double> gb;
+    rh_dev<unsigned long long> d_len;
+    RH_TRY(gb.alloc(7 * c->ng_pad));
+    RH_TRY(d_len.alloc(1));
+    RH_HIP(hipMemsetAsync(gb, 0, sizeof(double) * 7 * (size_t)c->ng_pad, c->stream));
+    RH_HIP(hipMemsetAsync(d_len, 0, sizeof(unsigned long long), c->stream));
+    RH_HIP(hipMemsetAsync(c->pl_gb32, 0, sizeof(float) * 8 * (size_t)c->ng_pad, c->stream));
+    RH_HIP(hipMemsetAsync(c->pl_gm32, 0, sizeof(uint32_t) * 4 * (size_t)c->ng_pad, c->stream));
+    RH_TRY(rhk_group_bounds_of(c, c->pl_sub, c->s_pad, c->s, c->ngroups, gb, c->ng_pad));
+    hipLaunchKernelGGL(gb32_kernel, dim3(cdiv4(c->ngroups, 256)), dim3(256), 0, c->stream, gb, c->ng_pad, c->ngroups, c->pl_gb32);
+    hipLaunchKernelGGL(nsig_kernel, dim3(cdiv4(c->ngroups, 4)), dim3(256), 0, c->stream, c->pl_sub, c->s_pad, c->s, c->ngroups, c->pl_gm32, d_len);
+    hipLaunchKernelGGL(st32_kernel, dim3(cdiv4(c->nst, 64)), dim3(64), 0, c->stream, gb, c->ng_pad, c->ngroups, S4_STG, c->nst, c->pl_st32);
+    hipLaunchKernelGGL(nsig_st_kernel, dim3(cdiv4(c->nst, 64)), dim3(64), 0, c->stream, c->pl_gm32, c->ngroups, S4_STG, c->nst, c->pl_stm32);
+    RH_HIP(hipGetLastError());
+    RH_HIP(hipStreamSynchronize(c->stream));
+    return RH_OK;
+}
+
+#ifndef RH_PLANE_ORDER_MIN_TILES
+#define RH_PLANE_ORDER_MIN_TILES 256
+#endif
+static bool plane_order_wanted(const rh_cloud *c)
+{
+    if (c->pl_sub == nullptr) return false;
+    const int64_t opt = rh_opt_int(c, RH_OPT_PLANE_ORDER, 0);
+    return opt == 1 || (opt == 0 && (c->ngroups + S4_TG - 1) / S4_TG >= RH_PLANE_ORDER_MIN_TILES);
+}
+
 static inline int64_t stlist_bytes(const rh_cloud *c, int64_t cap) { return (int64_t)sizeof(uint16_t) * c->nst * 4 * cap; }
 static int ensure_stlists(rh_cloud *c, rh_batch_ws &w, int64_t cap)
 {
@@ -1007,16 +1044,24 @@
         return RH_E_INTERNAL;
     }
     const int dbg = (int)rh_opt_int(c, RH_OPT_G2_DBG, 0);
+    const bool nsig_on = on_subset && c->gm32 != nullptr && rh_opt_int(c, RH_OPT_NSIG, 0) != 2;
     S4AllArgs A;
     for (int k = 0; k < 4; k++)
-        A.k[k] = { (const rh_cls *)B.cls[k], B.box[k], B.prep[k], B.orig[k], job.nk[k], job.en[k], job.eps[k], job.cosa[k] };
+        A.k[k] = { (const rh_cls *)B.cls[k], B.box[k], B.prep[k], B.orig[k], job.nk[k], job.en[k], job.eps[k], job.cosa[k],
+                   PS.pts, PS.stride, PS.gb32, nsig_on ? (const uint32_t *)c->gm32 : nullptr };
+    const bool plane_on = on_subset && d_masks_int == nullptr && dbg == 0 && plane_order_wanted(c) &&
+                          (job.en[RH_PLANE] == nullptr || job.en[RH_PLANE] == c->sub_enabled.get());
+    if (plane_on) {
+        S4KindArgs &P = A.k[RH_PLANE];
+        P.pts = c->pl_sub;
+        P.gb32 = c->pl_gb32;
+        if (nsig_on) P.gm32 = c->pl_gm32;
+        if (P.en != nullptr) P.en = c->pl_enabled;
+    }
     A.stop = job.stop;
     A.ntiles = ntiles;
     A.bstride = job.bstride;
     A.ngroups = PS.ngroups;
-    A.gb32 = PS.gb32;
-    const bool nsig_on = on_subset && c->gm32 != nullptr && rh_opt_int(c, RH_OPT_NSIG, 0) != 2;
-    A.gm32 = nsig_on ? (const uint32_t *)c->gm32 : nullptr;
     A.masks = d_masks_int;
     A.occ = d_masks_int ? w.d_occ : nullptr;
     A.mstride = d_masks_int ? w.mstride4 : 0;
@@ -1047,7 +1092,8 @@
     if (use_lists) {
         StCullArgs SA;
         for (int k = 0; k < 4; k++) { SA.box[k] = B.box[k]; SA.nk[k] = job.nk[k]; }
-        SA.bstride = job.bstride; SA.stcap = w.stlist_cap; SA.st32 = c->st32; SA.stm32 = nsig_on && c->stm32 != nullptr ? (const uint32_t *)c->stm32 : nullptr; SA.stlist = w.d_stlist; SA.stcount = w.d_stcount;
+        SA.bstride = job.bstride; SA.stcap = w.stlist_cap; SA.st32 = c->st32; SA.st32_plane = plane_on ? c->pl_st32 : c->st32;
+        SA.stm32 = nsig_on && c->stm32 != nullptr ? (const uint32_t *)(plane_on ? c->pl_stm32 : c->stm32) : nullptr; SA.stlist = w.d_stlist; SA.stcount = w.d_stcount;
         hipLaunchKernelGGL(st_cull_kernel, dim3((unsigned)c->nst, 4), dim3(256), 0, c->stream, SA);
         A.stlist = w.d_stlist; A.stcount = w.d_stcount; A.stcap = w.stlist_cap;
         if (job.ev_listed != nullptr) RH_HIP(hipEventRecord(job.ev_listed, c->stream));
@@ -1079,11 +1125,11 @@
     auto launch_tail = [&](unsigned ny) {
         const dim3 gt(tiles_x, ny);
         if (f32cloud) {
-            if (R == 4) hipLaunchKernelGGL((score4_kernel<4, false, true, true>), gt, dim3(64 * S4_W), 0, c->stream, PS.pts, PS.stride, PS.s, A, d_counts, dbg);
-            else hipLaunchKernelGGL((score4_kernel<8, false, true, true>), gt, dim3(64 * S4_W), 0, c->stream, PS.pts, PS.stride, PS.s, A, d_counts, dbg);
+            if (R == 4) hipLaunchKernelGGL((score4_kernel<4, false, true, true>), gt, dim3(64 * S4_W), 0, c->stream, PS.s, A, d_counts, dbg);
+            else hipLaunchKernelGGL((score4_kernel<8, false, true, true>), gt, dim3(64 * S4_W), 0, c->stream, PS.s, A, d_counts, dbg);
         } else {
-            if (R == 4) hipLaunchKernelGGL((score4_kernel<4, false, false, true>), gt, dim3(64 * S4_W), 0, c->stream, PS.pts, PS.stride, PS.s, A, d_counts, dbg);
-            else hipLaunchKernelGGL((score4_kernel<8, false, false, true>), gt, dim3(64 * S4_W), 0, c->stream, PS.pts, PS.stride, PS.s, A, d_counts, dbg);
+            if (R == 4) hipLaunchKernelGGL((score4_kernel<4, false, false, true>), gt, dim3(64 * S4_W), 0, c->stream, PS.s, A, d_counts, dbg);
+            else hipLaunchKernelGGL((score4_kernel<8, false, false, true>), gt, dim3(64 * S4_W), 0, c->stream, PS.s, A, d_counts, dbg);
         }
     };
     if (loop_max > 0 && d_masks_int == nullptr && nchunks <= loop_max) {
@@ -1093,8 +1139,8 @@
     }
 #define RH_S4_LAUNCH(RR, MM, FF)                                                                                                              \
     do {                                                                                                                                      \
-        if (use_lists) hipLaunchKernelGGL((score4_kernel<RR, MM, FF, false, true>), grid, dim3(64 * S4_W), 0, c->stream, PS.pts, PS.stride, PS.s, A, d_counts, dbg); \
-        else hipLaunchKernelGGL((score4_kernel<RR, MM, FF>), grid, dim3(64 * S4_W), 0, c->stream, PS.pts, PS.stride, PS.s, A, d_counts, dbg);  \
+        if (use_lists) hipLaunchKernelGGL((score4_kernel<RR, MM, FF, false, true>), grid, dim3(64 * S4_W), 0, c->stream, PS.s, A, d_counts, dbg); \
+        else hipLaunchKernelGGL((score4_kernel<RR, MM, FF>), grid, dim3(64 * S4_W), 0, c->stream, PS.s, A, d_counts, dbg);  \
     } while (0)
 #define RH_S4_LAUNCH_R(MM, FF)                                                                                         \
     do {                                                                                                               \
@@ -1225,8 +1271,22 @@
     RH_TRY(d_o.alloc(72));
     RH_HIP(hipMemcpyAsync(d_c, h.data(), sizeof(S4SoundCand) * (size_t)b, hipMemcpyHostToDevice, c->stream));
     RH_HIP(hipMemsetAsync(d_o, 0, sizeof(unsigned long long) * 72, c->stream));
-    hipLaunchKernelGGL(cls_sound_kernel, dim3((unsigned)c->ngroups, (unsigned)std::min<int32_t>(b, 64)), dim3(64), 0, c->stream, c->sub, c->s_pad, c->s,
-                       c->gb32, c->st32, c->tile32, c->gm32, c->stm32, d_c, b, A, d_o);
+    const bool pl = plane_order_wanted(c);
+    const dim3 grid((unsigned)c->ngroups, (unsigned)std::min<int32_t>(b, 64));
+    hipLaunchKernelGGL(cls_sound_kernel, grid, dim3(64), 0, c->stream, c->sub, c->s_pad, c->s, c->gb32, c->st32, c->tile32, c->gm32, c->stm32, d_c, b, A,
+                       pl ? 0xe : 0xf, d_o);
+    rh_dev<double> pl_gb;
+    rh_dev<float> pl_tile32;
+    if (pl) {
+        RH_TRY(pl_gb.alloc(7 * c->ng_pad));
+        RH_TRY(pl_tile32.alloc(8 * std::max<int64_t>(1, c->ntile)));
+        RH_HIP(hipMemsetAsync(pl_gb, 0, sizeof(double) * 7 * (size_t)c->ng_pad, c->stream));
+        RH_TRY(rhk_group_bounds_of(c, c->pl_sub, c->s_pad, c->s, c->ngroups, pl_gb, c->ng_pad));
+        hipLaunchKernelGGL(st32_kernel, dim3(cdiv4(c->ntile, 64)), dim3(64), 0, c->stream, pl_gb, c->ng_pad, c->ngroups, S4_TG, c->ntile, pl_tile32);
+        hipLaunchKernelGGL(cls_sound_kernel, grid, dim3(64), 0, c->stream, c->pl_sub, c->s_pad, c->s, c->pl_gb32, c->pl_st32, pl_tile32, c->pl_gm32, c->pl_stm32, d_c,
+                           b, A, 0x1, d_o);
+    }
+    RH_HIP(hipGetLastError());
     unsigned long long ho[72];
     RH_HIP(hipMemcpyAsync(ho, d_o, sizeof ho, hipMemcpyDeviceToHost, c->stream));
     RH_HIP(hipStreamSynchronize(c->stream));
```

After: 85.90 million candidates/s, median of 6. 4.3% higher.
